# jnsquire/sregex

Hardware: AMD Instinct MI355X
Metric: GB/s input scanned (whole job), gen-data stream resident in HBM (higher is better)
Workload: dtype u8; 1 GPU; configs[1]: /[a-z]+@[a-z]+\.[a-z]+/ Pike first-match + captures; 1 stream x 4.00 GiB gen-data (abccc.. + 'aaabbccb'); bytes_per_gpu=4294967293, streams_per_gpu=1, segment_bytes=16896, fixup_rounds=0, matches=0, engine=scan, lineage_passes=0, world_size=1

## Files before the change

sregex_amd/csrc/sre_hip_batch.cpp:

```cpp
#include <sregex_hip.h>
#include "sre_hip_runtime.h"
#include "sre_hip_scan.h"
#include "sre_scan_host.h"
#include "sre_dfa.h"
#include "sre_nfa.h"
#include "sre_hip_nfa.h"
#include "sre_nfa_wide.h"
#include "sre_hip_nfa_wide.h"
#include "sre_pwave.h"
#include "sre_hip_lines.h"
#include "sre_lines_gather.h"
#include "sre_lines_route.h"
#include "sre_lines_route_key.h"
#include "sre_lines_sort.h"
#include "sre_lines_sort_text.h"
#include "sre_lines_tally.h"
#include "sre_lines_tally_top.h"
#include "sre_lines_distinct.h"
#include "sre_lines_sums.h"
#include "sre_lines_keyset.h"
#include "sre_lines_join.h"
#include "sre_hip_streams.h"
#include "sre_streams_nfa.h"
#include <stddef.h>
#include <stdio.h>
#include <stdlib.h>
#include <string.h>
#include <atomic>
#include <chrono>
#include <initializer_list>
#include <vector>

#define SRE_SPECULATIVE_FIXUPS 2

struct sre_hip_scanner_s {
    sre_program_t     *prog;
    sre_hip_program_s *dp;
    int                mode, engine;
    char               kernel_name[64];
    uint32_t           ovec_slots;
    size_t             cap_streams;
    const void       **d_ptrs;
    uint64_t          *d_lens;
    int64_t           *d_records;
    void              *d_ctx;
    size_t             ctx_stride, ctx_cap;
    uint64_t          *h_lens;
    const void       **h_ptrs;
    size_t             last_n;
    hipStream_t        last_stream;
    sre_dfa_t                *dfa;
    sre_scan_device_tables_t *tab;
    uint32_t                  seg_override;
    uint64_t                  seg_cap_env;
    sre_scan_geom_t           geom;
    uint64_t                 *d_seg_first, *h_seg_first;
    sre_seg_summary_t        *d_sum;
    sre_seg_digest_t         *d_digest;
    size_t                    sum_cap;
    sre_stream_status_t      *d_status, *h_status;
    void                     *d_acc;
    int64_t                  *d_lo, *h_lo;
    uint16_t                 *d_scratch;
    size_t                    scratch_cap;
    sre_seg_lineage_t        *d_maps, *d_blocks;
    size_t                    maps_cap;
    uint8_t                  *d_fn;
    size_t                    fn_cap;
    int                       exact_passes;
    int                       lineage_passes;
    uint32_t                  next_init_variant;
    int                       blocks_per_cu;
    hipStream_t               tail_stream;
    bool                      tail_stream_set;
    int                       fixup_rounds;
    hipEvent_t                ev0, ev1;
    int                       ev_valid;
    sre_int_t                *h_records;
    hipEvent_t                ev_done;
    uint64_t                 *d_in, *h_in;
    unsigned char            *d_out, *h_out;
    sre_nfa_t                *nfa;
    sre_nfa_tables_t          ntab;
    sre_nfa_sa_tables_t       satab;
    bool                      use_sa;
    sre_nfa_wide_t           *wnfa;
    sre_nfa_wide_tables_t     wtab;
    uint64_t                 *d_wsets;
    bool                      wide_kernel;
    struct NfaCount          *cnt;
    uint8_t                  *d_sflags, *h_sflags;
    sre_nfa_count_req_t      *d_creq, *h_creq;
    size_t                    cnt_cap;
    int                       count_rounds;
    sre_pwave_hdr_t          *h_pwave;
    void                     *d_pwave;
    size_t                    layout_n;
    sre_nfa_summary_t        *d_nsum;
    size_t                    nsum_cap;
    uint64_t                 *d_belief;
    uint8_t                  *d_bvalid;
    uint64_t                 *d_nmat;
    size_t                    nmat_cap;
    void                     *d_nacc;
    sre_nfa_status_t         *d_nstatus, *h_nstatus;
    const uint64_t           *d_eset;
    uint64_t                 *d_ends;
    size_t                    ends_cap;
    uint64_t                 *d_lblk;
    size_t                    lblk_cap;
    int64_t                  *d_rows;
    size_t                    rows_cap;
    sre_lines_info_t         *d_linfo, *h_linfo;
    bool                      last_lines;
    int                       line_batches;
    double                    lines_kernel_ms;
    bool                      lines_device;
    size_t                    short_lines;
    hipEvent_t                ev_l0, ev_l1;
    uint64_t                 *d_fval;
    size_t                    fval_cap;
    uint64_t                 *d_fblk;
    size_t                    fblk_cap;
    uint64_t                 *d_cbits;
    size_t                    cbits_cap;
    uint64_t                 *d_cblk;
    size_t                    cblk_cap;
    uint64_t                 *d_fstart;
    size_t                    fstart_cap;
    uint8_t                  *d_lit;
    uint8_t                  *h_lit;
    size_t                    lit_len;
    bool                      lit_valid;
    uint64_t                 *d_rcnt;
    size_t                    rcnt_cap;
    uint64_t                 *d_rval;
    size_t                    rval_cap;
    uint64_t                 *d_rmeta;
    size_t                    rmeta_cap;
    int32_t                  *d_rmap;
    int32_t                  *h_rmap;
    bool                      rmap_valid;
    uint64_t                 *d_rres, *h_rres;
    uint64_t                 *d_ttab;
    size_t                    ttab_cap;
    uint32_t                 *d_tslot;
    size_t                    tslot_cap;
    uint64_t                 *d_vval;
    size_t                    vval_cap;
    uint64_t                 *d_vstart;
    size_t                    vstart_cap;
    sre_ls_agg_t             *d_vcopy;
    size_t                    vcopy_cap;
    int64_t                  *d_jkey;
    size_t                    jkey_cap;
    uint64_t                 *d_kitem[2];
    size_t                    kitem_cap[2];
    int8_t                   *d_sclass;
    size_t                    sclass_cap;
    uint32_t                 *d_sline[2];
    size_t                    sline_cap[2];
    uint64_t                 *d_pcount;
    size_t                    pcount_cap;
    sre_ls_agg_t             *d_psums;
    size_t                    psums_cap;
    uint64_t                 *d_pfirst;
    size_t                    pfirst_cap;
    uint32_t                 *d_pinv;
    size_t                    pinv_cap;
    uint64_t                 *d_pstart;
    size_t                    pstart_cap;
};

struct NfaCountStream {
    const uint8_t *base;
    uint64_t       n;
    uint64_t       cur;
    uint64_t       q;
    uint64_t       horizon;
    uint32_t       var_cur, var_q, mode_q;
    int64_t        count;
    bool           done, error;
    std::vector<sre_int_t> last;
};
struct NfaCount {
    std::vector<NfaCountStream> st;
    std::vector<size_t>         active;
};

static void
scanner_release(void *data)
{
    sre_hip_scanner_t *sc = static_cast<sre_hip_scanner_t *>(data);
    delete sc->cnt;
    free(sc->h_pwave);
    if (sc->d_pwave) (void) hipFree(sc->d_pwave);
    if (sc->d_sflags) (void) hipFree(sc->d_sflags);
    if (sc->h_sflags) (void) hipHostFree(sc->h_sflags);
    if (sc->d_creq) (void) hipFree(sc->d_creq);
    if (sc->h_creq) (void) hipHostFree(sc->h_creq);
    if (sc->d_in) (void) hipFree(sc->d_in);
    if (sc->h_in) (void) hipHostFree(sc->h_in);
    if (sc->d_out) (void) hipFree(sc->d_out);
    if (sc->h_out) (void) hipHostFree(sc->h_out);
    if (sc->d_ctx) (void) hipFree(sc->d_ctx);
    if (sc->d_sum) (void) hipFree(sc->d_sum);
    if (sc->d_digest) (void) hipFree(sc->d_digest);
    if (sc->d_acc) (void) hipFree(sc->d_acc);
    if (sc->d_lo) (void) hipFree(sc->d_lo);
    if (sc->h_lo) (void) hipHostFree(sc->h_lo);
    if (sc->d_scratch) (void) hipFree(sc->d_scratch);
// ... 569 lines not shown

static uint64_t
scan_seg_knobs(sre_hip_scanner_t *sc)
{
    uint64_t seg = sc->seg_override;
    const char *e = getenv("SRE_HIP_SEG_BYTES");
    if (seg == 0 && e && atoi(e) > 0 && atoi(e) % 256 == 0) seg = (uint64_t) atoi(e);
    e = getenv("SRE_HIP_SEG_CAP");
    sc->seg_cap_env = e && atoi(e) > 0 ? (uint64_t) atoi(e) : 0;
    return seg;
}

static uint64_t
nfa_seg_knobs(sre_hip_scanner_t *sc)
{
    uint64_t seg = scan_seg_knobs(sc);
    const char *e = getenv("SRE_HIP_SEG_BYTES");
    if (seg == 0 && e && atoi(e) > 0 && atoi(e) % 64 == 0) seg = (uint64_t) atoi(e);
    return seg;
}

static uint64_t
scan_seg_cap(const sre_hip_scanner_t *sc)
{
    return sc->seg_cap_env ? sc->seg_cap_env : 40960;
}

static int
scan_events(sre_hip_scanner_t *sc)
{
    if (sc->ev0 == NULL) {
        SRE_HIP_TRY(hipEventCreate(&sc->ev0));
        SRE_HIP_TRY(hipEventCreate(&sc->ev1));
    }
    return 0;
hip_failed:
    return -1;
}

static void
call_begin(sre_hip_scanner_t *sc)
{
    sc->last_lines = false;
    sc->fixup_rounds = 0;
    sc->exact_passes = 0;
    sc->lineage_passes = 0;
    sc->ev_valid = 0;
}

static void
geom_clear(sre_hip_scanner_t *sc)
{
    sc->geom = sre_scan_geom_t();
    sc->d_eset = NULL;
}

static void
geom_device(sre_hip_scanner_t *sc, uint64_t n, uint64_t seg, uint64_t nsegs)
{
    geom_clear(sc);
    sc->geom.streams = reinterpret_cast<const uint8_t *const *>(sc->d_ptrs);
    sc->geom.lens = sc->d_lens;
    sc->geom.seg_first = sc->d_seg_first;
    sc->geom.nstreams = (uint32_t) n;
    sc->geom.seg_bytes = (uint32_t) seg;
    sc->geom.nsegs = nsegs;
}

static uint64_t
scan_resident(sre_hip_scanner_t *sc)
{
    if (sc->blocks_per_cu == 0) {
        sc->blocks_per_cu = sc->engine == SRE_HIP_ENGINE_NFA
                                ? (sc->wide_kernel ? sre_nfa_wide_blocks_per_cu(&sc->wtab)
                                   : sc->use_sa ? sre_nfa_sa_blocks_per_cu(&sc->satab)
                                              : sre_nfa_blocks_per_cu(sc->mode == SRE_HIP_THOMPSON ? 0 : 1, sc->ntab.nslices,
                                                                      sc->ntab.nassert != 0))
                                                             : sre_scan_blocks_per_cu(&sc->tab->h);
    }
    return (uint64_t) sre_hip_cu_count() * (uint64_t) sc->blocks_per_cu * SRE_SCAN_BLOCK;
}

static int scan_buffers(sre_hip_scanner_t *sc, size_t nstreams, uint64_t seg, uint64_t nsegs);

static int
nfa_buffers(sre_hip_scanner_t *sc, uint64_t nsegs)
{
    if (nsegs > sc->nsum_cap) {
        if (sc->d_nsum) (void) hipFree(sc->d_nsum);
        if (sc->d_belief) (void) hipFree(sc->d_belief);
        if (sc->d_bvalid) (void) hipFree(sc->d_bvalid);
        if (sc->d_wsets) (void) hipFree(sc->d_wsets);
        sc->d_nsum = NULL;
        sc->d_belief = NULL;
        sc->d_bvalid = NULL;
        sc->d_wsets = NULL;
        sc->nsum_cap = 0;
        SRE_HIP_TRY(hipMalloc(reinterpret_cast<void **>(&sc->d_nsum), nsegs * sizeof(sre_nfa_summary_t)));
        SRE_HIP_TRY(hipMalloc(reinterpret_cast<void **>(&sc->d_belief), nsegs * nfa_words(sc) * sizeof(uint64_t)));
        if (sc->wide_kernel) SRE_HIP_TRY(hipMalloc(reinterpret_cast<void **>(&sc->d_wsets), nsegs * 2 * nfa_words(sc) * sizeof(uint64_t)));
        SRE_HIP_TRY(hipMalloc(reinterpret_cast<void **>(&sc->d_bvalid), nsegs));
        sc->nsum_cap = nsegs;
    }
    return 0;
hip_failed:
    return -1;
}

static int
scan_geometry(sre_hip_scanner_t *sc, size_t nstreams, uint32_t init_variant, uint32_t flags, uint32_t entry_state)
{
    uint64_t total = 0;
    for (size_t i = 0; i < nstreams; i++) total += sc->h_lens[i];
    uint64_t seg = scan_seg_knobs(sc);
    if (seg == 0) {
        const uint64_t resident = scan_resident(sc);
        seg = sre_scan_auto_segment(total, resident, scan_seg_cap(sc));
    }
    uint64_t nsegs = 0;
    for (size_t i = 0; i < nstreams; i++) {
        sc->h_seg_first[i] = nsegs;
        uint64_t k = (sc->h_lens[i] + seg - 1) / seg;
        nsegs += k ? k : 1;
    }
    sc->h_seg_first[nstreams] = nsegs;
    geom_clear(sc);
    sc->geom.streams = reinterpret_cast<const uint8_t *const *>(sc->d_ptrs);
    sc->geom.lens = sc->d_lens;
    sc->geom.seg_first = sc->d_seg_first;
    sc->geom.nstreams = (uint32_t) nstreams;
    sc->geom.seg_bytes = (uint32_t) seg;
    sc->geom.nsegs = nsegs;
    sc->geom.init_variant = init_variant;
    sc->geom.entry_state = entry_state;
    sc->geom.one_ptr = static_cast<const uint8_t *>(sc->h_ptrs[0]);
    sc->geom.one_len = sc->h_lens[0];
    sc->geom.flags = flags | ((nstreams == 1 && sc->engine == SRE_HIP_ENGINE_SCAN) ? SRE_GEOM_ONE : 0u);

    if (sc->engine == SRE_HIP_ENGINE_NFA) return nfa_buffers(sc, nsegs);
    return scan_buffers(sc, nstreams, seg, nsegs);
}

static int
scan_buffers(sre_hip_scanner_t *sc, size_t nstreams, uint64_t seg, uint64_t nsegs)
{
    if (nsegs > sc->sum_cap) {
        if (sc->d_sum) (void) hipFree(sc->d_sum);
        sc->d_sum = NULL;
        sc->sum_cap = 0;
        SRE_HIP_TRY(hipMalloc(reinterpret_cast<void **>(&sc->d_sum), nsegs * sizeof(sre_seg_summary_t)));
        sc->sum_cap = nsegs;
    }
    sc->geom.digest = NULL;
    if (nsegs <= SRE_VERIFY_ONE_SEGS && sc->mode != SRE_HIP_PIKE_COUNT) {
        if (sc->d_digest == NULL
            && hipMalloc(reinterpret_cast<void **>(&sc->d_digest), SRE_VERIFY_ONE_SEGS * sizeof(sre_seg_digest_t)) != hipSuccess)
        {
            sc->d_digest = NULL;
        }
        sc->geom.digest = sc->d_digest;
    }
    {
        size_t need = nstreams * ((size_t) seg + 16);
        if (need > sc->scratch_cap) {
            if (sc->d_scratch) (void) hipFree(sc->d_scratch);
            sc->d_scratch = NULL;
            sc->scratch_cap = 0;
            SRE_HIP_TRY(hipMalloc(reinterpret_cast<void **>(&sc->d_scratch), need * sizeof(uint16_t)));
            sc->scratch_cap = need;
        }
    }
    return 0;
hip_failed:
    return -1;
}

static int
nfa_windows(sre_hip_scanner_t *sc, const int64_t *d_lo, const sre_nfa_count_req_t *d_creq, hipStream_t stream)
{
    const uint32_t n = sc->geom.nstreams;
    if (sc->d_pwave) {
        SRE_HIP_TRY(sre_launch_pike_window_wave(sc->d_pwave, sc->h_pwave, sc->d_ptrs, sc->d_lens, n, sc->d_records,
                                                sc->ovec_slots, reinterpret_cast<sre_nfa_window_t *>(sc->d_nstatus), d_lo,
                                                d_creq, stream));
    } else {
        SRE_HIP_TRY(sre_launch_pike_window(sc->dp->d_blob, sc->dp->blob_bytes, sc->d_ptrs, sc->d_lens, n, sc->d_ctx, sc->ctx_stride,
                                           sc->d_records, sc->ovec_slots,
                                           reinterpret_cast<sre_nfa_window_t *>(sc->d_nstatus), d_lo,
                                           d_creq, stream));
    }
    return 0;
hip_failed:
    return -1;
}

static int
nfa_finish(sre_hip_scanner_t *sc, const int64_t *d_lo, const sre_nfa_count_req_t *d_creq, hipStream_t stream)
{
    const int kmode = sc->mode == SRE_HIP_THOMPSON ? SRE_HIP_THOMPSON : SRE_HIP_PIKE_FIRST;
    if (sc->wide_kernel) {
        SRE_HIP_TRY(sre_launch_nfa_wide_verify(kmode, sc->wtab.W, sc->geom, sc->d_nsum, sc->d_wsets, sc->d_nacc, sc->d_nstatus,
                                               sc->d_belief, sc->d_bvalid, sc->d_records, sc->ovec_slots, d_lo, stream));
    } else {
        SRE_HIP_TRY(sre_launch_nfa_verify(kmode, sc->geom, sc->d_nsum, sc->d_nacc, sc->d_nstatus,
                                          sc->d_belief, sc->d_bvalid, sc->d_records, sc->ovec_slots, d_lo, stream));
    }
    if (sc->mode != SRE_HIP_THOMPSON) return nfa_windows(sc, d_lo, d_creq, stream);
    return 0;
hip_failed:
    return -1;
}

static uint64_t
count_horizon(uint64_t dflt)
{
    const char *e = getenv("SRE_HIP_COUNT_HORIZON");
    return e && atoll(e) > 0 ? (uint64_t) atoll(e) : dflt;
}

static int
nfa_enqueue_pass(sre_hip_scanner_t *sc, size_t nstreams, uint32_t init_variant, const uint8_t *d_sflags,
                 const sre_nfa_count_req_t *d_creq, hipStream_t stream)
{
    if (scan_geometry(sc, nstreams, init_variant, 0, 0) != 0) return -1;
    sc->geom.sflags = d_sflags;
    SRE_HIP_TRY(hipMemcpyAsync(sc->d_in, sc->h_in, (3 * sc->layout_n + 1) * sizeof(uint64_t),
                               hipMemcpyHostToDevice, stream));
    if (scan_events(sc) != 0) return -1;
    {
        const bool timed = !sc->ev_valid;
        if (timed) SRE_HIP_TRY(hipEventRecord(sc->ev0, stream));
        SRE_HIP_TRY(nfa_launch_scan(sc, NULL, NULL, NULL, stream));
        if (timed) SRE_HIP_TRY(hipEventRecord(sc->ev1, stream));
        sc->ev_valid = 1;
    }
    if (sc->tail_stream_set && sc->tail_stream != stream) {
        SRE_HIP_TRY(hipStreamWaitEvent(sc->tail_stream, sc->ev1, 0));
        stream = sc->tail_stream;
    }
    return nfa_finish(sc, NULL, d_creq, stream);
hip_failed:
    return -1;
}

static int
nfa_fixup_round(sre_hip_scanner_t *sc, const sre_nfa_count_req_t *d_creq, hipStream_t stream)
{
    if (++sc->fixup_rounds > 1000000) {
        fprintf(stderr, "[sregex-hip] NFA scanner fix-up did not converge\n");
        return -1;
    }
    if (sc->fixup_rounds > SRE_SPECULATIVE_FIXUPS && sc->geom.nsegs <= ((size_t) 1 << 23)
        && getenv("SRE_HIP_NO_NFA_EXACT") == NULL) {
        if (sc->wide_kernel) {
            const size_t need = sre_nfa_wide_matrix_bytes(sc->wtab.W, sc->geom.nsegs);
            if (need > sc->nmat_cap * 64 * sizeof(uint64_t)) {
                if (sc->d_nmat) (void) hipFree(sc->d_nmat);
                sc->d_nmat = NULL;
                sc->nmat_cap = 0;
                size_t free_b = 0, total_b = 0;
                if (hipMemGetInfo(&free_b, &total_b) == hipSuccess && need <= free_b / 2
                    && hipMalloc(reinterpret_cast<void **>(&sc->d_nmat), need) == hipSuccess) {
                    sc->nmat_cap = need / (64 * sizeof(uint64_t));
                } else {
                    (void) hipGetLastError();
                    sc->d_nmat = NULL;
                }
            }
            if (sc->d_nmat) {
                SRE_HIP_TRY(sre_launch_nfa_wide_exact_entries(sc->wtab, sc->geom, sc->d_nsum, sc->d_wsets, sc->d_lo, sc->d_nmat,
                                                              sc->d_belief, sc->d_bvalid, stream));
                sc->exact_passes++;
            }
        } else {
            if (sc->geom.nsegs > sc->nmat_cap) {
                if (sc->d_nmat) (void) hipFree(sc->d_nmat);
                sc->d_nmat = NULL;
                sc->nmat_cap = 0;
                SRE_HIP_TRY(hipMalloc(reinterpret_cast<void **>(&sc->d_nmat), sc->geom.nsegs * 64 * sizeof(uint64_t)));
                sc->nmat_cap = sc->geom.nsegs;
            }
            SRE_HIP_TRY(sre_launch_nfa_exact_entries(sc->use_sa ? 1 : 0, sc->ntab, sc->satab, sc->geom, sc->d_nsum, sc->d_lo,
                                                     sc->d_nmat, sc->d_belief, sc->d_bvalid, stream));
            sc->exact_passes++;
        }
    }
    SRE_HIP_TRY(nfa_launch_scan(sc, sc->d_lo, sc->d_belief, sc->d_bvalid, stream));
    return nfa_finish(sc, sc->d_lo, d_creq, stream);
hip_failed:
    return -1;
}

static int
nfa_settle(sre_hip_scanner_t *sc, size_t n, const sre_nfa_count_req_t *d_creq, hipStream_t stream, bool *psettled)
{
    for (bool first = true;; first = false) {
        if (!first) {
            SRE_HIP_TRY(hipMemcpyAsync(sc->h_nstatus, sc->d_nstatus, n * sizeof(sre_nfa_status_t),
                                       hipMemcpyDeviceToHost, stream));
            SRE_HIP_TRY(hipStreamSynchronize(stream));
        }
        size_t pending = 0;
        for (size_t i = 0; i < n; i++) {
            if (sc->h_nstatus[i].done) {
                sc->h_lo[i] = -1;
            } else {
                sc->h_lo[i] = sc->h_nstatus[i].first_bad;
                pending++;
            }
        }
        if (pending == 0) break;
// ... 240 lines not shown
    return -1;
}

typedef uint64_t sre_lines_info_t::*LinfoWord;
#define LINFO(word) (&sre_lines_info_t::word)

static hipError_t
linfo_read(sre_hip_scanner_t *sc, hipStream_t stream, std::initializer_list<LinfoWord> words)
{
    const char *base = reinterpret_cast<const char *>(sc->h_linfo);
    size_t      lo = sizeof(sre_lines_info_t), hi = 0;
    for (LinfoWord w : words) {
        const size_t at = (size_t) (reinterpret_cast<const char *>(&(sc->h_linfo->*w)) - base);
        lo = at < lo ? at : lo;
        hi = at + sizeof(uint64_t) > hi ? at + sizeof(uint64_t) : hi;
    }
    return hipMemcpyAsync(reinterpret_cast<char *>(sc->h_linfo) + lo, reinterpret_cast<const char *>(sc->d_linfo) + lo, hi - lo,
                          hipMemcpyDeviceToHost, stream);
}

static int
lines_status_counters(sre_hip_scanner_t *sc, size_t n, hipStream_t stream)
{
    SRE_HIP_TRY(sre_launch_lines_settle(sc->d_status, (uint32_t) n, sc->d_linfo, stream));
    SRE_HIP_TRY(linfo_read(sc, stream, {LINFO(pending), LINFO(maps)}));
    SRE_HIP_TRY(hipStreamSynchronize(stream));
    return 0;
hip_failed:
    return -1;
}

static int
scan_settle(sre_hip_scanner_t *sc, size_t n, hipStream_t stream, bool with_captures, bool *psettled,
            bool counters = false)
{
    bool settled = true;
    int  batch = sc->mode == SRE_HIP_PIKE_COUNT ? 2 : SRE_SPECULATIVE_FIXUPS + 1;
    for (;;) {
        size_t pending = 0;
        if (counters) pending = (size_t) sc->h_linfo->pending;
        else for (size_t i = 0; i < n; i++) pending += sc->h_status[i].done ? 0 : 1;
        if (pending == 0) break;
        settled = false;
        for (int r = 0; r < batch; r++) {
            if (++sc->fixup_rounds > 1000000) {
                fprintf(stderr, "[sregex-hip] scanner fix-up did not converge\n");
                return -1;
            }
            const uint8_t *d_entry = NULL;
            static const bool count_exact = getenv("SRE_HIP_NO_COUNT_EXACT") == NULL;
            if ((sc->mode != SRE_HIP_PIKE_COUNT || count_exact) && sc->fixup_rounds > SRE_SPECULATIVE_FIXUPS) {
                if (sc->geom.nsegs > sc->fn_cap) {
                    if (sc->d_fn) (void) hipFree(sc->d_fn);
                    sc->d_fn = NULL;
                    sc->fn_cap = 0;
                    const size_t nchunks = sc->geom.nsegs / 256 + 1;
                    SRE_HIP_TRY(hipMalloc(reinterpret_cast<void **>(&sc->d_fn),
                                          sc->geom.nsegs * 64 + nchunks * 64 + nchunks + sc->geom.nsegs + 64));
                    sc->fn_cap = sc->geom.nsegs;
                }
                const size_t nchunks = sc->geom.nsegs / 256 + 1;
                uint8_t *d_comp = sc->d_fn + sc->geom.nsegs * 64, *d_chunk = d_comp + nchunks * 64;
                uint8_t *d_ent = d_chunk + nchunks;
                SRE_HIP_TRY(sre_launch_exact_entries(sc->tab->d_tab, sc->tab->h, sc->geom, sc->d_sum, sc->d_status,
                                                     sc->d_fn, d_comp, d_chunk, d_ent, stream));
                d_entry = d_ent;
                sc->exact_passes++;
            }
            SRE_HIP_TRY(sre_launch_scan(sc->tab->d_tab, sc->tab->h, sc->geom, sc->d_sum, sc->d_status, d_entry, stream));
            SRE_HIP_TRY(sre_launch_verify(sc->tab->h, sc->geom, sc->d_sum, sc->d_acc, sc->d_status, stream));
            if (with_captures) {
                SRE_HIP_TRY(sre_launch_captures(sc->tab->d_tab, sc->tab->h, sc->geom, sc->d_sum,
                                                sc->d_status, sc->d_scratch, sc->d_records,
                                                sc->ovec_slots, NULL, NULL, 0, 0, stream));
            }
        }
        if (counters) {
            if (lines_status_counters(sc, n, stream) != 0) return -1;
        } else {
            SRE_HIP_TRY(hipMemcpyAsync(sc->h_status, sc->d_status, n * sizeof(sre_stream_status_t),
                                       hipMemcpyDeviceToHost, stream));
            SRE_HIP_TRY(hipStreamSynchronize(stream));
        }
        batch = sc->mode == SRE_HIP_PIKE_COUNT ? (batch < 16 ? 2 * batch : 16) : 1;
    }
    if (psettled) *psettled = settled;
    return 0;
hip_failed:
    return -1;
}

static int
scan_lineage_pass(sre_hip_scanner_t *sc, hipStream_t stream)
{
    if (sc->geom.nsegs > sc->maps_cap) {
        if (sc->d_maps) (void) hipFree(sc->d_maps);
        if (sc->d_blocks) (void) hipFree(sc->d_blocks);
        sc->d_maps = sc->d_blocks = NULL;
        sc->maps_cap = 0;
        SRE_HIP_TRY(hipMalloc(reinterpret_cast<void **>(&sc->d_maps),
                              sc->geom.nsegs * sizeof(sre_seg_lineage_t)));
        SRE_HIP_TRY(hipMalloc(reinterpret_cast<void **>(&sc->d_blocks),
                              (sc->geom.nsegs / SRE_LINEAGE_BLOCK + 1) * sizeof(sre_seg_lineage_t)));
        sc->maps_cap = sc->geom.nsegs;
    }
    sc->lineage_passes++;
    SRE_HIP_TRY(sre_launch_lineage(sc->tab->d_tab, sc->tab->h, sc->geom, sc->d_sum,
                                   sc->d_status, sc->d_maps, sc->d_blocks, stream));
    SRE_HIP_TRY(sre_launch_captures(sc->tab->d_tab, sc->tab->h, sc->geom, sc->d_sum,
                                    sc->d_status, sc->d_scratch, sc->d_records,
                                    sc->ovec_slots, sc->d_maps, sc->d_blocks,
                                    1, 0, stream));
    return 0;
hip_failed:
    return -1;
}

extern "C" SRE_API int
sre_hip_scan_results(sre_hip_scanner_t *sc, sre_int_t *results)
{
    if (sc->last_lines) return -1;
    if (sc->last_n == 0) return 0;
    const size_t n = sc->last_n;
    hipStream_t  stream = sc->last_stream;

    const size_t bytes = n * (2 + (size_t) sc->ovec_slots) * sizeof(int64_t);
    bool         settled = true;

    if (sc->engine == SRE_HIP_ENGINE_NFA && sc->cnt != NULL) return nfa_count_rounds(sc, results);
    SRE_HIP_TRY(hipEventSynchronize(sc->ev_done));
    if (sc->engine == SRE_HIP_ENGINE_NFA && nfa_settle(sc, n, NULL, stream, &settled) != 0) return -1;
    if (sc->engine == SRE_HIP_ENGINE_SCAN) {
        if (scan_settle(sc, n, stream, true, &settled) != 0) return -1;
        if (sc->mode != SRE_HIP_THOMPSON) {
            size_t want = 0;
            for (size_t i = 0; i < n; i++) want += sc->h_status[i].need_maps != 0;
            if (want) {
                settled = false;
                if (scan_lineage_pass(sc, stream) != 0) return -1;
            }
        }
    }
    if (sc->engine == SRE_HIP_ENGINE_SCAN && getenv("SRE_HIP_DEBUG_STATUS")) {
        for (size_t i = 0; i < n && i < 8; i++) {
            const sre_stream_status_t &t = sc->h_status[i];
            fprintf(stderr, "[sregex-hip] stream %zu: rc %lld count %lld ev_pos %lld ev_sp %lld ev_state %u ev_sym %u "
                            "ev_apos %lld ev_astate %u ev_seg %lld limit %lld need_maps %d seg %u\n",
                    i, (long long) t.rc, (long long) t.count, (long long) t.ev_pos, (long long) t.ev_sp,
                    t.ev_state, t.ev_sym, (long long) t.ev_apos, t.ev_astate, (long long) t.ev_seg,
                    (long long) t.limit, t.need_maps, sc->geom.seg_bytes);
        }
        const size_t ns = sc->geom.nsegs < 16 ? (size_t) sc->geom.nsegs : 16;
        std::vector<sre_seg_summary_t> hs(ns);
        if (hipMemcpy(hs.data(), sc->d_sum, ns * sizeof(sre_seg_summary_t), hipMemcpyDeviceToHost) == hipSuccess) {
            for (size_t k = 0; k < ns; k++) {
                fprintf(stderr, "[sregex-hip]   seg %zu: s_in %x s_out %x flags %x count %lld cur_sp %lld term %lld "
                                "pe_pos %lld lm_pos %lld lm_sp %lld\n",
                        k, hs[k].s_in, hs[k].s_out, hs[k].flags, (long long) hs[k].count,
                        (long long) hs[k].cur_sp, (long long) hs[k].term_pos, (long long) hs[k].pe_pos,
                        (long long) hs[k].lm_pos, (long long) hs[k].lm_sp);
            }
        }
    }
    if (!settled) {
        SRE_HIP_TRY(hipMemcpyAsync(sc->h_records, sc->d_records, bytes, hipMemcpyDeviceToHost, stream));
        if (sc->engine == SRE_HIP_ENGINE_NFA) {
            SRE_HIP_TRY(hipMemcpyAsync(sc->h_nstatus, sc->d_nstatus, n * sizeof(sre_nfa_status_t),
                                       hipMemcpyDeviceToHost, stream));
        }
        SRE_HIP_TRY(hipStreamSynchronize(stream));
    }
    memcpy(results, sc->h_records, bytes);
    return 0;
hip_failed:
    return -1;
}

extern "C" SRE_API int
sre_hip_scan_batch(sre_hip_scanner_t *sc, const void *const *d_streams, const size_t *lens,
    size_t nstreams, sre_int_t *results, void *hip_stream)
{
    if (sre_hip_scan_enqueue(sc, d_streams, lens, nstreams, hip_stream) != 0) return -1;
    return sre_hip_scan_results(sc, results);
}


template <typename T>
static int
lines_grow(T **p, size_t *cap, size_t bytes)
{
    if (bytes <= *cap) return 0;
    if (*p) (void) hipFree(*p);
    *p = NULL;
    *cap = 0;
    SRE_HIP_TRY(hipMalloc(reinterpret_cast<void **>(p), bytes));
    *cap = bytes;
    return 0;
hip_failed:
    return -1;
}

static uint64_t
lines_batch_limit(void)
{
    const char     *e = getenv("SRE_HIP_LINES_BATCH");
    const long long v = e ? atoll(e) : 0;
    return v > 0 ? (v < (1ll << 24) ? (uint64_t) v : (uint64_t) 1 << 24) : SRE_LINES_BATCH;
}

static int
lines_split(sre_hip_scanner_t *sc, const void *d_buf, size_t len, int delim, hipStream_t stream, uint64_t *pn)
{
    *pn = 0;
    if (len == 0) return 0;
    const uint64_t head = reinterpret_cast<uintptr_t>(d_buf) & 15u;
    const uint64_t ntiles = (head + len + SRE_LINES_TILE_BYTES - 1) / SRE_LINES_TILE_BYTES;
    const uint64_t nblk = (lines_batch_limit() + SRE_LINES_ITEMS - 1) / SRE_LINES_ITEMS + 1;
    if (lines_grow(&sc->d_lblk, &sc->lblk_cap, (ntiles > nblk ? ntiles : nblk) * sizeof(uint64_t)) != 0) return -1;
    SRE_HIP_TRY(sre_launch_lines_count(d_buf, len, (uint32_t) delim, sc->d_lblk, sc->d_linfo, stream));
    SRE_HIP_TRY(hipMemcpyAsync(&sc->h_linfo->nlines, &sc->d_linfo->nlines, sizeof(uint64_t), hipMemcpyDeviceToHost, stream));
    SRE_HIP_TRY(hipStreamSynchronize(stream));
    if (lines_grow(&sc->d_ends, &sc->ends_cap, sc->h_linfo->nlines * sizeof(uint64_t)) != 0) return -1;
    SRE_HIP_TRY(sre_launch_lines_write(d_buf, len, (uint32_t) delim, sc->d_lblk, sc->d_ends, stream));
    *pn = sc->h_linfo->nlines;
    return 0;
hip_failed:
    return -1;
}

struct LinesSink {
    int        delim;
    void      *d_out;
    size_t     out_cap;
    sre_int_t *d_index;
    size_t     index_cap;
    int        mode;
    const sre_extract_groups_t *groups;
    int                         fsep;
    const sre_subst_pieces_t   *pieces;
    bool                        route;
    uint32_t                    nreg;
    const sre_extract_groups_t *vgroups;
    bool                        context;
    const uint64_t             *d_cbits;
    uint32_t                    join;
    const void                 *d_dict;
};

static bool
sink_open(LinesSink *sink, const sre_hip_scanner_t *sc, const void *d_buf, size_t len, int delim, int flags, void *d_out,
          size_t out_cap, sre_int_t *d_index, size_t index_cap)
{
    if (sc == NULL || delim < 0 || delim > 255 || (out_cap != 0 && d_out == NULL) || (index_cap != 0 && d_index == NULL)
        || (len != 0 && d_buf == NULL))
    {
        return false;
    }
    if (len != 0 && out_cap != 0) {
        const uintptr_t b = reinterpret_cast<uintptr_t>(d_buf), o = reinterpret_cast<uintptr_t>(d_out);
        if (o < b + len && b < o + out_cap) return false;
    }
    *sink = LinesSink();
    sink->delim = sink->fsep = delim;
    sink->mode = (flags & SRE_HIP_LINES_ALL) ? 2 : (flags & SRE_HIP_LINES_INVERT) ? 1 : 0;
    sink->d_out = d_out;
    sink->out_cap = out_cap;
    sink->d_index = d_index;
    sink->index_cap = index_cap;
    return true;
}

static bool
sink_first_match(const sre_hip_scanner_t *sc, const char *call, const char *reads)
{
    if (sc->mode == SRE_HIP_PIKE_FIRST) return true;
    fprintf(stderr, "[sregex-hip] %s: the scanner's mode must be SRE_HIP_PIKE_FIRST (the first match's %s)\n", call, reads);
    return false;
}

static bool
sink_groups(const sre_hip_scanner_t *sc, const int *groups, size_t ngroups, sre_extract_groups_t *gr)
{
    memset(gr, 0, sizeof(*gr));
    gr->k = (uint32_t) ngroups;
    for (size_t f = 0; f < ngroups; f++) {
        if (groups[f] < 0 || groups[f] > 0xFFFF || 2 * (size_t) groups[f] + 1 >= (size_t) sc->ovec_slots) return false;
        gr->g[f] = (uint16_t) groups[f];
    }
    return true;
}

static uint32_t
sink_entries(const LinesSink *sink)
{
    return sink->pieces ? sink->pieces->np + 2 : sink->groups ? sink->groups->k : sink->join ? sink->join : 1;
}

static int
sink_select(sre_hip_scanner_t *sc, const LinesSink *sink, uint32_t slots, uint64_t nmax, uint64_t i0, hipStream_t stream)
{
    const int64_t          *recs = sc->d_records;
    const uint64_t         *ends = sc->d_ends;
    const sre_lines_info_t *li = sc->d_linfo;
    uint64_t               *val = sc->d_fval, *start = sc->d_fstart;
    const int               all = sink->mode == 2;
    if (sink->route) SRE_HIP_TRY(sre_launch_route_select(recs, slots, nmax, i0, sink->nreg, sc->d_rmap, ends, li, val, stream));
    else if (sink->pieces) SRE_HIP_TRY(sre_launch_subst_select(recs, slots, nmax, i0, all, sink->pieces, ends, li, val, start, stream));
// ... 2187 lines not shown
```

sregex_amd/csrc/sre_hip_scan.h:

```cpp
#ifndef SRE_HIP_SCAN_H
#define SRE_HIP_SCAN_H

#include <hip/hip_runtime.h>
#include <stdint.h>

#define SRE_CEILING_GRID   2048

#include "sre_scan_fast.h"

#define SRE_SCAN_MAX_SHADOWS  2u
#define SRE_SCAN_MAX_ROWS(bits)   ((65536u - 768u - ((bits) == 8 ? 512u : (8u / (bits)) * 512u)) / 1024u)
#define SRE_SCAN_MAX_STATES       62u
#define SRE_SCAN_BLOCK        256u
#define SRE_SCAN_LDS_LIMIT    (128u * 1024u)
#define SRE_CAPTURE_MAX_GRID   16384u
#define SRE_CAPTURE_LANE_STREAMS 4096u
#define SRE_CAPTURE_LDS_LIMIT  (144u * 1024u)
#define SRE_SCAN_ROUND        64u
#define SRE_SCAN_LINE         128u
#define SRE_SCAN_SEG_ALIGN    256u

#define SRE_SCAN_NINIT 4u
#define SRE_DEV_EV_DONE_EMPTY 3
#define SRE_DEV_EV_POP_FULL   4

typedef struct {
    uint32_t next;
    uint8_t  kind;
    uint8_t  src;
    uint16_t regex;
    uint32_t lin_off;
    uint16_t lin_n;
    uint8_t  skipped;
    uint8_t  pad;
    uint64_t saves;
    uint64_t early;
} sre_dev_trans_t;

typedef struct {
    uint32_t nstates, ncls, nslots, max_threads;
    uint32_t init[4];
    uint32_t word_restart;
    int32_t  mode;
    uint32_t fast_bytes;
    uint32_t stride, class_bits;
    const uint32_t        *fast;
    const uint32_t        *fast_plain;
    const uint8_t         *cls;
    const sre_dev_trans_t *trans;
    const uint16_t        *trans2;
    const uint8_t         *lin_parent;
    const uint64_t        *lin_saves;
    const uint64_t        *lin_early;
    const uint8_t         *lin_flags;
    uint32_t               lin_total, list_total;
    const uint8_t         *state_flags;
    const uint32_t        *list_off;
    const uint32_t        *list_pcs;
    const uint32_t        *multi_ncaps;
    uint32_t nregexes;
    uint32_t any_fresh;
    uint32_t nshadow;
    uint32_t fast_rows;
    uint32_t wide;
    uint8_t  shadow_state[SRE_SCAN_MAX_SHADOWS];
    const uint8_t         *unskip;
    const uint16_t        *neutral;
} sre_scan_tables_t;

typedef struct {
    uint32_t s_in;
    uint32_t s_out;
    uint32_t flags;
    uint32_t pad;
    uint32_t pe_state, pe_sym;
    int64_t  pe_pos, pe_sp;
    uint32_t lm_state, lm_sym;
    int64_t  lm_pos, lm_sp;
    int64_t  lm_apos, pe_apos;
    uint32_t lm_astate, pe_astate;
    int64_t  term_pos;
    int64_t  count;
    int64_t  cur_sp;
    int64_t  in_pe_pos;
    uint32_t in_pe_state, in_pe_sym;
    uint32_t stable_until, stable_from;
} sre_seg_summary_t;

typedef struct sre_seg_digest_s {
    uint32_t s_in, s_out, bits, count;
} sre_seg_digest_t;

#define SRE_SUM_PENDING   1u
#define SRE_SUM_TERM      2u
#define SRE_SUM_LASTEV    4u
#define SRE_SUM_ERROR     8u
#define SRE_SUM_IN_PENDING 16u
#define SRE_SUM_STABLE    32u

#define SRE_STATE_SKIP    0x40000000u

typedef struct {
    uint64_t anc;
    uint16_t saved;
    uint16_t stop;
    uint32_t pad;
} sre_seg_lineage_t;

#define SRE_LINEAGE_BLOCK  256u
#define SRE_WALK_BUDGET    256

#define SRE_STREAM_MAX_THREADS 64u
#define SRE_STREAM_MAX_SLOTS   64u
typedef struct {
    uint32_t state;
    uint32_t has_pending;
    int64_t  pending_regex;
    int64_t  pending_vec[SRE_STREAM_MAX_SLOTS];
    int64_t  caps[SRE_STREAM_MAX_THREADS][SRE_STREAM_MAX_SLOTS];
    int64_t  caps_next[SRE_STREAM_MAX_THREADS][SRE_STREAM_MAX_SLOTS];
} sre_stream_ctx_t;

#define SRE_VERIFY_ONE_SEGS 8192u
#define SRE_STREAM_UNSETTLED (-100)
#define SRE_STREAM_PENDING   (-101)

typedef struct {
    int64_t  rc;
    int64_t  has_pending, pending[2];
    int64_t  ev_in_chunk;
    int64_t  poisoned;
    int64_t  next_state;
    int64_t  ev_slot1;
    int64_t  ov[SRE_STREAM_MAX_SLOTS];
} sre_stream_result_t;

typedef struct {
    int64_t  first_bad;
    int64_t  limit;
    int64_t  count;
    int64_t  rc;
    int64_t  ev_pos, ev_sp;
    uint32_t ev_state, ev_sym;
    int64_t  ev_apos;
    uint32_t ev_astate;
    uint32_t valid_from;
    int64_t  ev_seg;
    int64_t  unst_seg;
    int64_t  unst_end;
    int32_t  done;
    int32_t  error;
    int32_t  need_maps;
    int32_t  pad;
} sre_stream_status_t;

typedef struct {
    const uint8_t *const *streams;
    const uint64_t *lens;
    const uint64_t *seg_first;
    uint32_t nstreams;
    uint32_t seg_bytes;
    uint64_t nsegs;
    uint32_t init_variant;
    uint32_t flags;
    uint32_t entry_state;
    const uint8_t *one_ptr;
    uint64_t one_len;
    const uint8_t *sflags;
    struct sre_seg_digest_s *digest;
    const uint32_t *sentry;
} sre_scan_geom_t;
#define SRE_SENTRY_STATE(e)   ((e) & 0xffffu)
#define SRE_SENTRY_CONTINUES  0x40000000u
#define SRE_SENTRY_NO_EOF     0x80000000u
#define SRE_SFLAG_INIT(f)    ((f) & 3u)
#define SRE_SFLAG_SNAP(f)    (((f) >> 2) & 3u)
#define SRE_SFLAG_MODE(f)    (((f) >> 4) & 1u)
#define SRE_SFLAG_NO_EOF     32u

#define SRE_GEOM_CONTINUES 1u
#define SRE_GEOM_NO_EOF    2u
#define SRE_GEOM_ONE       4u

#ifdef __HIPCC__
static __host__ __device__ inline uint64_t
sre_scan_auto_segment(uint64_t total, uint64_t resident, uint64_t seg_cap)
{
    uint64_t rounds = (total + resident * seg_cap - 1) / (resident * seg_cap);
    if (rounds < 1) rounds = 1;
    const uint64_t lanes = resident * rounds - (resident * rounds >> 6);
    uint64_t       seg = (total / lanes + SRE_SCAN_SEG_ALIGN) / SRE_SCAN_SEG_ALIGN * SRE_SCAN_SEG_ALIGN;
    if (seg < 256) seg = 256;
    if (seg % 4096 == 0) seg += SRE_SCAN_SEG_ALIGN;
    return seg;
}

static __device__ inline const uint8_t *
geom_ptr(const sre_scan_geom_t &G, uint32_t s)
{
    return (G.flags & SRE_GEOM_ONE) ? G.one_ptr : G.streams[s];
}
static __device__ inline uint64_t
geom_len(const sre_scan_geom_t &G, uint32_t s)
{
    return (G.flags & SRE_GEOM_ONE) ? G.one_len : G.lens[s];
}
static __device__ inline uint64_t
geom_first(const sre_scan_geom_t &G, uint32_t i)
{
    return (G.flags & SRE_GEOM_ONE) ? (i ? G.nsegs : 0) : G.seg_first[i];
}
#endif

#ifdef __cplusplus
extern "C" {
#endif
hipError_t sre_launch_gen_data(void *d_dst, uint64_t n, uint64_t tail_len, const void *d_tail,
    hipStream_t stream);
hipError_t sre_launch_read_ceiling(const void *d_src, uint64_t n, uint32_t *d_sink,
    hipStream_t stream);
hipError_t sre_launch_read_pattern(const void *d_src, uint64_t n, uint32_t seg_bytes,
    uint32_t tile, uint32_t lds_bytes, uint32_t *d_sink, hipStream_t stream);

size_t sre_scan_lds_bytes(const sre_scan_tables_t *h_tab);
int sre_scan_blocks_per_cu(const sre_scan_tables_t *h_tab);

hipError_t sre_launch_scan(const sre_scan_tables_t *d_tab, sre_scan_tables_t h_tab,
    sre_scan_geom_t geom, sre_seg_summary_t *d_sum, const sre_stream_status_t *d_lo, const uint8_t *d_entry,
    hipStream_t stream);
hipError_t sre_launch_exact_entries(const sre_scan_tables_t *d_tab, sre_scan_tables_t h_tab,
    sre_scan_geom_t geom, const sre_seg_summary_t *d_sum, const sre_stream_status_t *d_status,
    uint8_t *d_fn, uint8_t *d_comp, uint8_t *d_chunk_entry, uint8_t *d_entry, hipStream_t stream);
hipError_t sre_launch_stream_tail(const sre_scan_tables_t *d_tab, sre_scan_tables_t h_tab,
    sre_scan_geom_t geom, const sre_seg_summary_t *d_sum, sre_stream_status_t *d_status,
    uint16_t *d_scratch, sre_stream_ctx_t *d_ctx, sre_stream_result_t *result, int64_t base, int eof,
    uint32_t ovec_slots, int verify, hipStream_t stream);
hipError_t sre_launch_upload_words(const uint64_t *h_src_mapped, uint64_t *d_dst, uint32_t nwords, hipStream_t stream);
size_t sre_scan_verify_acc_bytes(uint32_t nstreams);
hipError_t sre_scan_verify_acc_init(void *d_acc, uint32_t nstreams, hipStream_t stream);
hipError_t sre_launch_verify(sre_scan_tables_t h_tab, sre_scan_geom_t geom,
    const sre_seg_summary_t *d_sum, void *d_acc, sre_stream_status_t *d_status,
    hipStream_t stream);
hipError_t sre_launch_captures(const sre_scan_tables_t *d_tab, sre_scan_tables_t h_tab,
    sre_scan_geom_t geom, const sre_seg_summary_t *d_sum, sre_stream_status_t *d_status,
    uint16_t *d_scratch, int64_t *d_records, uint32_t ovec_slots,
    const sre_seg_lineage_t *d_maps, const sre_seg_lineage_t *d_blocks, int use_maps,
    int verify, hipStream_t stream);
hipError_t sre_launch_lineage(const sre_scan_tables_t *d_tab, sre_scan_tables_t h_tab,
    sre_scan_geom_t geom, const sre_seg_summary_t *d_sum, const sre_stream_status_t *d_status,
    sre_seg_lineage_t *d_maps, sre_seg_lineage_t *d_blocks, hipStream_t stream);
#ifdef __cplusplus
// ... 4 lines not shown
```

sregex_amd/csrc/sre_hip_scan.hip:

```cpp
#include <hip/hip_runtime.h>
#include <stdlib.h>
#include "sre_hip_scan.h"
#include "sre_hip_streams.h"
#include "sre_hip_tile.h"

#define SRE_HIP_PIKE_COUNT 2
#define EV_DONE 1
#define EV_POP  2
#define RC_DECLINED (-5)
#define RC_ERROR    (-1)


__global__ void
sre_k_gen_data(uint8_t *__restrict__ dst, uint64_t n, uint64_t body, const uint8_t *__restrict__ tail)
{
    const uint64_t stride = (uint64_t) gridDim.x * blockDim.x * 16;
    for (uint64_t base = ((uint64_t) blockIdx.x * blockDim.x + threadIdx.x) * 16; base < n;
         base += stride)
    {
        uint8_t  v[16];
        unsigned ph = (unsigned) (base % 5);
#pragma unroll
        for (int k = 0; k < 16; k++) {
            uint64_t i = base + k;
// ... 302 lines not shown
            const bool    empty = w.ev_kind == EV_POP || w.ev_kind == SRE_DEV_EV_DONE_EMPTY;
            const int64_t e = pop ? w.ev_pos : w.ev_pos + 1;
            w.complete_match();
            if (empty) {
                if (e >= w.n) {
                    w.term_pos = p;
                    w.fl |= F_FINISHED;
                    return;
                }
                w.cur_sp = e + 1;
            } else {
                w.cur_sp = e;
            }
            w.st = T.init[restart_variant_of(T, byte_at(w.cur_sp - 1))];
            p = w.cur_sp;
            if (p > p_to && p_to <= w.n) w.fl |= F_SKIP_NEXT;
            w.anchor_pos = -1;
        }
    }
}

struct SpanResult {
    int64_t  sp;
    int64_t  last_pos, last_sp;
    uint32_t last_state, last_sym;
    int64_t  pend_pos;
    uint32_t pend_state, pend_sym;
};

__device__ __attribute__((noinline)) SpanResult
resolve_fast_span(const sre_scan_tables_t *Tp, const uint16_t *tr2, const uint8_t *data, int64_t gpos,
                  uint32_t len, uint32_t s0, int64_t sp0, int64_t pend0_pos, uint32_t pend0_state, uint32_t pend0_sym)
{
    const sre_scan_tables_t &T = *Tp;
    SpanResult r;
    uint32_t   st = s0;
    r.sp = sp0;
    r.last_pos = r.last_sp = -1;
    r.last_state = r.last_sym = 0;
    r.pend_pos = pend0_pos;
    r.pend_state = pend0_state;
    r.pend_sym = pend0_sym;
    for (uint32_t b = 0; b < len; b++) {
        const uint32_t         sym = T.cls[data[gpos + b]];
        const uint32_t t2 = tr2[st * (T.ncls + 1) + sym];
        struct { uint32_t next; uint8_t kind; } tr = {t2 & 0xffu, (uint8_t) (t2 >> 8)};
        if (tr.kind && tr.next == 0) {
            const bool pop = tr.kind == SRE_DEV_EV_POP_FULL && gpos + b > 0;
            r.last_pos = gpos + b;
            r.last_state = st;
            r.last_sym = sym;
            r.last_sp = r.sp;
            r.sp = pop ? gpos + b : gpos + b + 1;
            r.pend_pos = -1;
            st = T.init[restart_variant(T, data, r.sp)];
            if (pop) st = tr2[st * (T.ncls + 1) + sym] & 0xffu;
        } else if (tr.kind) {
            r.pend_pos = gpos + b;
            r.pend_state = st;
            r.pend_sym = sym;
            st = tr.next;
        } else if (tr.next == 0 && gpos + b > 0) {
            r.last_pos = r.pend_pos;
            r.last_state = r.pend_state;
            r.last_sym = r.pend_sym;
            r.last_sp = r.sp;
            r.sp = gpos + b;
            st = T.init[restart_variant(T, data, r.sp)];
            const uint32_t t3 = tr2[st * (T.ncls + 1) + sym];
            r.pend_pos = -1;
            if ((t3 >> 8) && (t3 & 0xffu) == 0) {
                r.last_pos = gpos + b;
                r.last_state = st;
                r.last_sym = sym;
                r.last_sp = r.sp;
                r.sp = gpos + b + 1;
                st = T.init[restart_variant(T, data, r.sp)];
            } else {
                if (t3 >> 8) {
                    r.pend_pos = gpos + b;
                    r.pend_state = st;
                    r.pend_sym = sym;
                }
                st = t3 & 0xffu;
            }
        } else {
            st = tr.next;
        }
    }
    return r;
}

template <int H>
__device__ inline uint32_t
add_w0_w(uint32_t a, uint32_t b)
{
    uint32_t r;
    if (H == 0) asm("v_add_u32_sdwa %0, %1, %2 dst_sel:DWORD dst_unused:UNUSED_PAD src0_sel:WORD_0 src1_sel:WORD_0" : "=v"(r) : "v"(a), "v"(b));
    if (H == 1) asm("v_add_u32_sdwa %0, %1, %2 dst_sel:DWORD dst_unused:UNUSED_PAD src0_sel:WORD_0 src1_sel:WORD_1" : "=v"(r) : "v"(a), "v"(b));
    if (H == 2) asm("v_add_u32_sdwa %0, %1, %2 dst_sel:DWORD dst_unused:UNUSED_PAD src0_sel:WORD_0 src1_sel:DWORD" : "=v"(r) : "v"(a), "v"(b));
    return r;
}

__device__ inline uint32_t
add_b3(uint32_t a, uint32_t b)
{
    uint32_t r;
    asm("v_add_u32_sdwa %0, %1, %2 dst_sel:DWORD dst_unused:UNUSED_PAD src0_sel:DWORD src1_sel:BYTE_3" : "=v"(r) : "v"(a), "v"(b));
    return r;
}

template <int K>
__device__ inline uint32_t
byte_x4(uint32_t v, uint32_t sh)
{
    uint32_t r;
    if (K == 0) asm("v_lshlrev_b32_sdwa %0, %1, %2 dst_sel:DWORD dst_unused:UNUSED_PAD src0_sel:DWORD src1_sel:BYTE_0" : "=v"(r) : "v"(sh), "v"(v));
    if (K == 1) asm("v_lshlrev_b32_sdwa %0, %1, %2 dst_sel:DWORD dst_unused:UNUSED_PAD src0_sel:DWORD src1_sel:BYTE_1" : "=v"(r) : "v"(sh), "v"(v));
    if (K == 2) asm("v_lshlrev_b32_sdwa %0, %1, %2 dst_sel:DWORD dst_unused:UNUSED_PAD src0_sel:DWORD src1_sel:BYTE_2" : "=v"(r) : "v"(sh), "v"(v));
    if (K == 3) asm("v_lshlrev_b32_sdwa %0, %1, %2 dst_sel:DWORD dst_unused:UNUSED_PAD src0_sel:DWORD src1_sel:BYTE_3" : "=v"(r) : "v"(sh), "v"(v));
    return r;
}

#ifdef SRE_NO_TAIL_PRIO
#define SRE_TAIL_PRIO() ((void) 0)
#else
#define SRE_TAIL_PRIO() __builtin_amdgcn_s_setprio(3)
#endif

#ifndef SRE_SCAN_PREFETCH
#define SRE_SCAN_PREFETCH 1
#endif
#ifndef SRE_SCAN_SPLIT_HOLD
#define SRE_SCAN_SPLIT_HOLD 3
#endif
constexpr int
scan_split_of(int mode, int bits, bool wide, bool grow)
{
#ifdef SRE_SCAN_SPLIT
    (void) mode; (void) bits; (void) wide; (void) grow;
    return SRE_SCAN_SPLIT;
#else
    if (mode != SRE_HIP_PIKE_COUNT) return (bits == 2 || bits == 4) ? 4 : 1;
    return (bits == 4 && !wide && grow) ? 4 : 1;
#endif
}
#ifndef SRE_FIRST_BLOCKS
#define SRE_FIRST_BLOCKS 4
#endif
#ifndef SRE_COUNT_BLOCKS
#define SRE_COUNT_BLOCKS 3
#endif

template <int MODE, int BITS, bool WIDE, bool GROW>
__global__ __launch_bounds__(SRE_SCAN_BLOCK, MODE == SRE_HIP_PIKE_COUNT ? SRE_COUNT_BLOCKS : SRE_FIRST_BLOCKS) void
sre_k_scan(const sre_scan_tables_t *__restrict__ tabp, sre_scan_geom_t G,
           sre_seg_summary_t *__restrict__ sum, const sre_stream_status_t *__restrict__ st_lo,
           const uint8_t *__restrict__ entry)
{
    constexpr int      TILE = SRE_SCAN_ROUND;
    constexpr int      WARM = SRE_SCAN_LINE;
    constexpr int      STRIDE = 8 / BITS;
    constexpr uint32_t ROWRAW = TILE / STRIDE * (WIDE ? 2 : 1);
    constexpr uint32_t ROWB = 2 * ROWRAW + 16;
    constexpr int      GIDX = 16 / STRIDE;
    typedef const __attribute__((address_space(3))) uint32_t *lds_u32_t;
    extern __shared__ __attribute__((aligned(16))) uint8_t lds[];
    __shared__ uint16_t clsx[BITS == 8 ? 1 : 8 / BITS][256];
    __shared__ sre_scan_tables_t Ts;

    const uint32_t tid = threadIdx.x;
    const uint32_t nst = tabp->nstates, nrows = tabp->fast_rows, nsh = tabp->nshadow;
    uint32_t *fast = reinterpret_cast<uint32_t *>(lds);
    uint8_t  *clsl = lds + nrows * SRE_FAST_ROW_BYTES;
    uint8_t  *trl = clsl + 256;
    const uint32_t tr_bytes = (nst * (tabp->ncls + 1) * 2u + 15u) & ~15u;
    uint8_t  *sfl = trl + tr_bytes;
    uint8_t  *tile = lds + (((size_t) (sfl - lds) + nst + 15u) & ~(size_t) 15u);
    RowDesc  *rows = reinterpret_cast<RowDesc *>(tile + SRE_SCAN_BLOCK * ROWB);
    (void) nrows;
    if (tid == 0) {
        Ts = *tabp;
        Ts.cls = clsl;
        Ts.state_flags = sfl;
    }
    constexpr uint32_t LDS_SLOW = 1u << 16;
    constexpr uint32_t LDS_CNT_SHIFT = 24;
    constexpr uint32_t LDS_FRESH = 1u << 17;
    const uint32_t fast_lds = (uint32_t) (uintptr_t) (__attribute__((address_space(3))) uint8_t *) lds;
    const uint32_t trap_lds = fast_lds + nst * SRE_FAST_ROW_BYTES;
    const uint32_t shadow_lds = trap_lds + SRE_FAST_ROW_BYTES;
    auto to_lds = [fast_lds, trap_lds](uint32_t g) -> uint32_t {
        if (g & SRE_FAST_SLOW) return trap_lds | LDS_SLOW;
        return (fast_lds + (g & ~(SRE_FAST_ROW_BYTES - 1)))
               | (((g >> SRE_FAST_CNT_SHIFT) & SRE_FAST_CNT_MASK) << LDS_CNT_SHIFT)
               | ((MODE == SRE_HIP_PIKE_COUNT && (g & SRE_FAST_EVT)) ? (128u << LDS_CNT_SHIFT) : 0u)
               | ((MODE == SRE_HIP_PIKE_COUNT && (g & SRE_FAST_NEXT_FRESH)) ? LDS_FRESH : 0u);
    };
    for (uint32_t i = tid; i < nst * 64; i += SRE_SCAN_BLOCK) {
        uint4 e = reinterpret_cast<const uint4 *>(tabp->fast)[i];
        e.x = to_lds(e.x);
        e.y = to_lds(e.y);
        e.z = to_lds(e.z);
        e.w = to_lds(e.w);
        reinterpret_cast<uint4 *>(fast)[i] = e;
    }
    fast[nst * 256 + tid] = trap_lds | LDS_SLOW;
    for (uint32_t q = 0; q < nsh; q++) {
        const uint32_t s = tabp->shadow_state[q], addr = shadow_lds + q * SRE_FAST_ROW_BYTES;
        const uint32_t gl = tabp->fast[s * 256 + tid];
        fast[(nst + 1 + q) * 256 + tid] = (gl & SRE_FAST_STABLE) ? addr : to_lds(gl);
    }
    for (uint32_t i = tid; i < nst * (tabp->ncls + 1); i += SRE_SCAN_BLOCK) {
        reinterpret_cast<uint16_t *>(trl)[i] = tabp->trans2[i];
    }
    for (uint32_t i = tid; i < tabp->nstates; i += SRE_SCAN_BLOCK) sfl[i] = tabp->state_flags[i];
    clsl[tid] = tabp->cls[tid];
    if (BITS != 8) {
#pragma unroll
        for (int u = 0; u < 8 / BITS; u++) clsx[u][tid] = (uint16_t) ((uint32_t) tabp->cls[tid] << (BITS * u + (WIDE ? 2 : 0)));
    }
    __syncthreads();
    const sre_scan_tables_t &T = Ts;

    const uint64_t g = (uint64_t) blockIdx.x * SRE_SCAN_BLOCK + tid;
    bool           active = g < G.nsegs;
    uint32_t       sidx = 0;
    uint64_t       k = 0;
    int64_t        lo_s = -2;
    if (active) {
        uint32_t a = 0, b = G.nstreams;
        while (b - a > 1) {
            uint32_t m = (a + b) >> 1;
            if (geom_first(G, m) <= g) a = m; else b = m;
        }
        sidx = a;
        k = g - geom_first(G, a);
        if (st_lo != nullptr) {
            lo_s = st_lo[sidx].done ? -1 : st_lo[sidx].first_bad;
            if (lo_s < 0 || (int64_t) k < lo_s) active = false;
        }
    }

    Walk w;
    w.T = &T;
    w.tr2 = reinterpret_cast<const uint16_t *>(trl);
    w.data = nullptr;
    w.n = 0;
    w.st = 0;
    w.ev_kind = 0;
    w.ev_state = w.ev_sym = 0;
    w.ev_pos = w.ev_sp = -1;
    w.ev_apos = -1;
    w.ev_astate = 0;
    w.cur_sp = -1;
    w.warm_lo = 0;
    w.anchor_pos = -1;
    w.anchor_state = 0;
    w.lm_state = w.lm_sym = 0;
    w.lm_pos = w.lm_sp = w.lm_apos = -1;
    w.lm_astate = 0;
    w.count = 0;
    w.term_pos = -1;
    w.fl = 0;

    int64_t  seg_a = 0, seg_b = 0;
    uint32_t s_in = 0, seed = 0;
    int64_t  in_pe_pos = -1;
    uint32_t in_pe_state = 0, in_pe_sym = 0;
    bool     last_seg = false, warm = false;
    RowDesc mine;
    mine.addr = 0;
    mine.lo = 0;
    mine.hi16 = -1;
    if (active) {
        w.data = geom_ptr(G, sidx);
        w.n = (int64_t) geom_len(G, sidx);
        seg_a = (int64_t) k * G.seg_bytes;
        seg_b = seg_a + G.seg_bytes;
        const uint64_t nseg = geom_first(G, sidx + 1) - geom_first(G, sidx);
        last_seg = (k + 1 == nseg);
        if (seg_b > w.n) seg_b = w.n;
        if (last_seg && G.sentry != nullptr && (G.sentry[sidx] & SRE_SENTRY_NO_EOF)) w.fl |= F_NO_EOF;

        if (k == 0) {
            w.st = G.sentry != nullptr ? SRE_SENTRY_STATE(G.sentry[sidx])
                   : (G.flags & SRE_GEOM_CONTINUES) ? G.entry_state : T.init[G.init_variant];
            w.cur_sp = 0;
        } else if (lo_s >= 0 && (int64_t) k == lo_s) {
            const sre_seg_summary_t &c = sum[g - 1];
            w.st = c.s_out & ~SRE_STATE_SKIP;
            w.set(F_SKIP_NEXT, MODE == SRE_HIP_PIKE_COUNT && (c.s_out & SRE_STATE_SKIP) != 0);
            w.cur_sp = c.cur_sp;
            if (c.flags & SRE_SUM_PENDING) {
                w.fl |= F_HAS_EV;
                w.ev_state = c.pe_state;
                w.ev_sym = c.pe_sym;
                w.ev_pos = c.pe_pos;
                w.ev_sp = c.pe_sp;
                w.ev_apos = c.pe_apos;
                w.ev_astate = c.pe_astate;
                w.ev_kind = (uint8_t) (w.tr2[c.pe_state * (T.ncls + 1) + c.pe_sym] >> 8);
                if (MODE == SRE_HIP_PIKE_COUNT) {
                    w.fl |= F_IN_PENDING;
                    in_pe_pos = c.pe_pos;
                    in_pe_state = c.pe_state;
                    in_pe_sym = c.pe_sym;
                }
            }
        } else if (entry != nullptr && entry[g] != 0xffu) {
            w.st = entry[g];
            if (MODE == SRE_HIP_PIKE_COUNT && lo_s > 0 && (T.state_flags[w.st] & 1)) {
                const sre_seg_summary_t &c = sum[geom_first(G, sidx) + lo_s - 1];
                if (c.flags & SRE_SUM_PENDING) {
                    w.fl |= F_HAS_EV | F_IN_PENDING;
                    w.ev_state = c.pe_state;
                    w.ev_sym = c.pe_sym;
                    w.ev_pos = c.pe_pos;
                    w.ev_sp = c.pe_sp;
                    w.ev_apos = -1;
                    w.ev_astate = 0;
                    w.ev_kind = (uint8_t) (w.tr2[c.pe_state * (T.ncls + 1) + c.pe_sym] >> 8);
                    in_pe_pos = c.pe_pos;
                    in_pe_state = c.pe_state;
                    in_pe_sym = c.pe_sym;
                }
            }
        } else {
            warm = true;
            seed = T.init[0];
            if (lo_s > 0) {
                const sre_seg_summary_t &c = sum[geom_first(G, sidx) + lo_s - 1];
                const uint32_t           cs = c.s_out & ~SRE_STATE_SKIP;
                if (cs != 0) {
                    if (!(MODE == SRE_HIP_PIKE_COUNT && (T.state_flags[cs] & 1))) {
                        seed = cs;
                    } else if (c.flags & SRE_SUM_PENDING) {
                        seed = cs;
                        w.fl |= F_HAS_EV;
                        w.ev_state = c.pe_state;
                        w.ev_sym = c.pe_sym;
                        w.ev_pos = c.pe_pos;
                        w.ev_sp = c.pe_sp;
                        w.ev_apos = -1;
                        w.ev_astate = 0;
                        w.ev_kind = (uint8_t) (w.tr2[c.pe_state * (T.ncls + 1) + c.pe_sym] >> 8);
                    }
                }
            }
            w.st = seed;
        }
        w.warm_lo = seg_a >= (int64_t) WARM ? seg_a - (int64_t) WARM : 0;
        s_in = w.st | (MODE == SRE_HIP_PIKE_COUNT && w.f(F_SKIP_NEXT) ? SRE_STATE_SKIP : 0u);
        mine.addr = (uint64_t) reinterpret_cast<uintptr_t>(w.data) + (uint64_t) (seg_a - WARM);
        mine.lo = warm ? (seg_a >= WARM ? 0 : (int32_t) (WARM - seg_a)) : WARM;
        mine.hi16 = (int32_t) (WARM + (seg_b - seg_a)) - 16;
    }
    rows[tid] = mine;

    int64_t  fcA_pos = -1, fcB_pos = -1, fc_sp0 = -1;
    uint32_t fcA_len = 0, fcA_s0 = 0, fcB_len = 0, fcB_s0 = 0;
    int64_t  lz_pos = -1;
    uint32_t lz_s0 = 0;
    auto note_span = [&](int64_t pos, uint32_t len, uint32_t s0, uint32_t cnt, bool warm_round) {
        w.fl &= ~F_HAS_EV;
        if (warm_round) return;
        if (w.f(F_SP_DIRTY)) {
            fcA_pos = fcB_pos;
            fcA_len = fcB_len;
            fcA_s0 = fcB_s0;
        } else {
            fc_sp0 = w.cur_sp;
            fcA_pos = -1;
        }
        fcB_pos = pos;
        fcB_len = len;
        fcB_s0 = s0;
        if (w.f(F_PEND_LAZY)) {
            fcB_pos = lz_pos;
            fcB_len = len + (w.f(F_LZ_GROUP) ? 16u : (uint32_t) TILE);
            fcB_s0 = lz_s0;
        }
        w.fl |= F_SP_DIRTY;
        w.count += cnt;
    };
    constexpr bool any_fresh = GROW;
    auto fast_span_done = [&](int64_t pos, uint32_t len, uint32_t s0, uint32_t sum, bool fresh1, bool warm_round) {
        if (!any_fresh) {
            if (sum) note_span(pos, len, s0, sum, warm_round);
            return;
        }
        if (sum == 0) {
            w.fl &= ~F_PEND_LAZY;
            return;
        }
        if (sum & 127u) note_span(pos, len, s0, sum & 127u, warm_round);
        else if (sum) w.fl &= ~F_HAS_EV;
        if (fresh1) {
            w.fl |= F_PEND_LAZY;
            w.set(F_LZ_GROUP, len == 16u);
            lz_pos = pos;
            lz_s0 = s0;
        } else {
            w.fl &= ~F_PEND_LAZY;
        }
    };
    auto settle = [&]() {
        if (MODE != SRE_HIP_PIKE_COUNT || !(w.fl & (F_SP_DIRTY | F_PEND_LAZY))) return;
        if (w.f(F_SP_DIRTY)) {
            int64_t sp0 = fc_sp0;
            if (fcA_pos >= 0) sp0 = resolve_fast_span(&T, w.tr2, w.data, fcA_pos, fcA_len, fcA_s0, -1, -1, 0, 0).sp;
            const SpanResult r = resolve_fast_span(&T, w.tr2, w.data, fcB_pos, fcB_len, fcB_s0, sp0, w.ev_pos, w.ev_state, w.ev_sym);
            if (r.last_pos >= 0) {
                w.fl |= F_LM_VALID;
                w.lm_pos = r.last_pos;
                w.lm_state = r.last_state;
                w.lm_sym = r.last_sym;
                w.lm_sp = r.last_sp;
                const bool anchored = r.last_sp < fcB_pos && r.last_pos - fcB_pos <= 256 && fcB_pos >= seg_a;
                w.lm_apos = anchored ? fcB_pos : (int64_t) -1;
                w.lm_astate = anchored ? fcB_s0 : 0u;
            }
            w.cur_sp = r.sp;
            w.fl &= ~F_SP_DIRTY;
        }
        if (w.f(F_PEND_LAZY)) {
            const SpanResult r = resolve_fast_span(&T, w.tr2, w.data, lz_pos, w.f(F_LZ_GROUP) ? 16u : (uint32_t) TILE, lz_s0,
                                                   -1, -1, 0, 0);
            w.fl &= ~F_PEND_LAZY;
            if (r.pend_pos >= 0) {
                w.fl |= F_HAS_EV;
                w.ev_pos = r.pend_pos;
                w.ev_state = r.pend_state;
                w.ev_sym = r.pend_sym;
                w.ev_kind = (uint8_t) (w.tr2[r.pend_state * (T.ncls + 1) + r.pend_sym] >> 8);
                w.ev_sp = w.cur_sp;
                const bool anchored = w.cur_sp < lz_pos && lz_pos >= seg_a;
                w.ev_apos = anchored ? lz_pos : (int64_t) -1;
                w.ev_astate = anchored ? lz_s0 : 0u;
            }
        }
    };

    constexpr uint32_t SU_UNSET = 0xffffffffu;
    uint32_t           su = SU_UNSET, run_off = 0;
    static_assert(SRE_SCAN_MAX_SHADOWS == 2, "two shadow rows");
    const uint32_t sh_st0 = nsh > 0 ? tabp->shadow_state[0] : 0xffffu, sh_st1 = nsh > 1 ? tabp->shadow_state[1] : 0xffffu;
    const uint32_t sh_ad0 = shadow_lds, sh_ad1 = shadow_lds + SRE_FAST_ROW_BYTES;
    const uint32_t     two = 2;
    (void) two;

    const uint32_t nrounds = WARM / TILE + G.seg_bytes / TILE;
    const uint32_t lag = (tid >> 5) & 1u;
    constexpr uint32_t DIST = SRE_SCAN_PREFETCH;
    constexpr int      NLOOK = TILE * BITS / 8;
    constexpr int      SPLIT = scan_split_of(MODE, BITS, WIDE, GROW);
    static_assert(SPLIT == 1 || SPLIT == 2 || SPLIT == 4, "SRE_SCAN_SPLIT is 1, 2 or 4");
    uint32_t           hold = 0;
    __syncthreads();
    auto round = [&](const uint32_t s, uint4 (&regs)[4]) __attribute__((always_inline)) {
        if (SPLIT > 1) {
            if (__builtin_amdgcn_ballot_w64((w.fl & F_SPLIT_MISS) != 0)) {
                hold = SRE_SCAN_SPLIT_HOLD;
                w.fl &= ~F_SPLIT_MISS;
            } else if (hold) {
                hold--;
            }
        }
        __builtin_amdgcn_fence(__ATOMIC_ACQ_REL, "wavefront");
        __builtin_amdgcn_wave_barrier();
        tile_store<BITS, WIDE>(regs, tile, clsx, tid, s);
        __builtin_amdgcn_fence(__ATOMIC_ACQ_REL, "wavefront");
        __builtin_amdgcn_wave_barrier();
        if (s + DIST <= nrounds) tile_fetch(regs, rows, tid, s + DIST);

        if (s < lag || s - lag >= nrounds) return;
        const uint32_t r = s - lag;
        const bool     warm_round = (r < WARM / TILE);
        if (!active || w.f(F_FINISHED) || (warm_round && !warm)) return;
        const int64_t base = seg_a - WARM + (int64_t) r * TILE;
        if (base >= seg_b || base < 0) return;
        w.anchor_pos = warm_round ? -1 : base;
        w.anchor_state = w.st;

        constexpr int ROWW = (ROWRAW + 3) / 4;
// ... 79 lines not shown
                        uint32_t nv = 1;
                        t = tc[0];
                        cnt = cc[0];
#pragma unroll
                        for (int c = 1; c < SPLIT; c++) {
                            if (nv == (uint32_t) c && ((t ^ t0) & 0xffffu) == 0) {
                                t = tc[c];
                                cnt += cc[c];
                                nv = c + 1;
                            }
                        }
                        if (!(t & LDS_SLOW)) {
#pragma unroll
                            for (int c = 1; c < SPLIT; c++) {
                                if (nv <= (uint32_t) c) serial(c * L, (c + 1) * L);
                            }
                        }
                    }
                }
            } else {
                serial(0, NLOOK);
            }
            if (!(t & LDS_SLOW)) {
                const uint32_t ridx = ((t & 0xffffu) - fast_lds) / SRE_FAST_ROW_BYTES;
                if (MODE == SRE_HIP_PIKE_COUNT) fast_span_done(base, TILE, w.st, cnt, (t & LDS_FRESH) != 0, warm_round);
                w.st = MODE == SRE_HIP_PIKE_COUNT ? ridx : ridx <= nst ? ridx : ridx == nst + 1 ? sh_st0 : sh_st1;
                if (MODE != SRE_HIP_PIKE_COUNT && w.f(F_SHADOW) && ridx <= nst) {
                    w.fl &= ~F_SHADOW;
                    if (su == SU_UNSET) su = (uint32_t) (base - seg_a);
                }
                if (r + 1 == WARM / TILE) {
                    s_in = w.st | (MODE == SRE_HIP_PIKE_COUNT && w.f(F_SKIP_NEXT) ? SRE_STATE_SKIP : 0u);
                    settle();
                    w.cur_sp = -1;
                    if (w.f(F_HAS_EV)) w.ev_sp = -1;
                    if (w.st == 0) w.fl |= F_FINISHED;
                    if (MODE == SRE_HIP_PIKE_COUNT) {
                        w.set(F_IN_PENDING, w.f(F_HAS_EV));
                        in_pe_pos = w.ev_pos;
                        in_pe_state = w.ev_state;
                        in_pe_sym = w.ev_sym;
                    }
                }
                return;
            }
        }
        if (MODE != SRE_HIP_PIKE_COUNT && !warm_round) {
            w.fl &= ~F_SHADOW;
            if (su == SU_UNSET) su = (uint32_t) (base - seg_a);
        }
#pragma unroll 1
        for (uint32_t q = 0; q < TILE / 16; q++) {
            const int64_t gp = base + q * 16;
            if (gp >= seg_b || w.f(F_FINISHED)) break;
            const int64_t g_end = gp + 16 <= seg_b ? gp + 16 : seg_b;
            bool          exact = (g_end != gp + 16) || (MODE == SRE_HIP_PIKE_COUNT && w.f(F_SKIP_NEXT));
            uint32_t      t = fast_lds + w.st * SRE_FAST_ROW_BYTES, cnt = 0;
            if (!exact) {
                constexpr int GW = GIDX * (WIDE ? 2 : 1) / 4;
                uint32_t      gw[GW];
                const uint32_t *gsrc = reinterpret_cast<const uint32_t *>(tile + tid * ROWB + (r & 1u) * ROWRAW) + q * GW;
#pragma unroll
                for (int x = 0; x < GW; x++) gw[x] = gsrc[x];
#pragma unroll
                for (int j = 0; j < GIDX; j++) {
                    const uint32_t ix = WIDE ? (gw[j >> 1] >> ((j & 1) * 16)) & 0xffffu
                                             : ((gw[j >> 2] >> ((j & 3) * 8)) & 0xffu) << 2;
                    t = *(lds_u32_t) (uintptr_t) ((t & 0xffffu) + ix);
                    if (MODE == SRE_HIP_PIKE_COUNT) cnt += t >> LDS_CNT_SHIFT;
                }
                exact = (t & LDS_SLOW) != 0;
            }
            if (exact) {
                settle();
                slow_run<MODE>(w, gp, g_end, warm_round, seed);
            } else {
                const uint32_t st1 = ((t & 0xffffu) - fast_lds) / SRE_FAST_ROW_BYTES;
                if (MODE == SRE_HIP_PIKE_COUNT) fast_span_done(gp, 16, w.st, cnt, (t & LDS_FRESH) != 0, warm_round);
                w.st = st1;
            }
        }
        if (r + 1 == WARM / TILE) {
            s_in = w.st | (MODE == SRE_HIP_PIKE_COUNT && w.f(F_SKIP_NEXT) ? SRE_STATE_SKIP : 0u);
            settle();
            w.cur_sp = -1;
            if (w.f(F_HAS_EV)) w.ev_sp = -1;
            if (w.st == 0) w.fl |= F_FINISHED;
            if (MODE == SRE_HIP_PIKE_COUNT) {
                w.set(F_IN_PENDING, w.f(F_HAS_EV));
                in_pe_pos = w.ev_pos;
                in_pe_state = w.ev_state;
                in_pe_sym = w.ev_sym;
            }
        }
    
    };
    uint4 regs[4];
    tile_fetch(regs, rows, tid, 0);
    if (DIST == 1) {
        for (uint32_t s = 0; s <= nrounds; s++) round(s, regs);
    } else {
        uint4 regs2[4];
        if (nrounds >= 1) tile_fetch(regs2, rows, tid, 1);
        for (uint32_t s = 0; s <= nrounds; s += 2) {
            round(s, regs);
            if (s + 1 <= nrounds) round(s + 1, regs2);
        }
    }

    if (!active) return;

    if (last_seg && !w.f(F_FINISHED) && !(G.flags & SRE_GEOM_NO_EOF) && !w.f(F_NO_EOF)) {
        settle();
        w.anchor_pos = -1;
        slow_run<MODE>(w, w.n, w.n + 1, false, 0);
    }
    settle();

    sre_seg_summary_t out;
    {
        const uint32_t seg_len = (uint32_t) (seg_b - seg_a);
        if (MODE == SRE_HIP_PIKE_COUNT || (w.f(F_FINISHED) && su == SU_UNSET)) su = 0;
        out.stable_until = su == SU_UNSET ? seg_len : su;
        out.stable_from = (MODE != SRE_HIP_PIKE_COUNT && w.f(F_SHADOW)) ? run_off : seg_len;
    }
    out.s_in = w.f(F_UNRESOLVED) ? 0xffffffffu : s_in;
    out.s_out = w.st | (MODE == SRE_HIP_PIKE_COUNT && w.f(F_SKIP_NEXT) ? SRE_STATE_SKIP : 0u);
    out.flags = 0;
    out.pad = 0;
    out.count = w.count;
    out.term_pos = w.term_pos;
    out.cur_sp = w.cur_sp;
    if (w.f(F_FINISHED) && w.term_pos >= 0) out.flags |= SRE_SUM_TERM;
    if (w.f(F_ERROR)) out.flags |= SRE_SUM_ERROR;
    if (w.f(F_HAS_EV)) out.flags |= SRE_SUM_PENDING;
    if (w.f(F_LM_VALID)) out.flags |= SRE_SUM_LASTEV;
    if (MODE == SRE_HIP_PIKE_COUNT && w.f(F_IN_PENDING)) out.flags |= SRE_SUM_IN_PENDING;
    if (MODE != SRE_HIP_PIKE_COUNT && out.stable_until == G.seg_bytes && !last_seg) out.flags |= SRE_SUM_STABLE;
    out.in_pe_pos = in_pe_pos;
    out.in_pe_state = in_pe_state;
    out.in_pe_sym = in_pe_sym;
    out.pe_state = w.ev_state;
    out.pe_sym = w.ev_sym;
    out.pe_pos = w.ev_pos;
    out.pe_sp = w.ev_sp;
    out.lm_state = w.lm_state;
    out.lm_sym = w.lm_sym;
    out.lm_pos = w.lm_pos;
    out.lm_sp = w.lm_sp;
    out.lm_apos = w.lm_apos;
    out.lm_astate = w.lm_astate;
    out.pe_apos = w.ev_apos;
    out.pe_astate = w.ev_astate;
    sum[g] = out;
    if (MODE != SRE_HIP_PIKE_COUNT && G.digest != nullptr) {
        sre_seg_digest_t dg;
        dg.s_in = out.s_in;
        dg.s_out = out.s_out;
        dg.bits = ((out.flags & SRE_SUM_TERM) ? 2u : 0u) | ((out.flags & SRE_SUM_LASTEV) ? 4u : 0u) | (out.cur_sp >= 0 ? 8u : 0u)
                  | ((out.flags & SRE_SUM_STABLE) ? 0u : 16u);
        dg.count = (uint32_t) out.count;
        G.digest[g] = dg;
    }
}


#define SRE_FN_CHUNK 256u

template <int BITS>
__global__ __launch_bounds__(256) void
sre_k_seg_functions(const sre_scan_tables_t *__restrict__ tabp, sre_scan_geom_t G,
                    const sre_stream_status_t *__restrict__ status, uint8_t *__restrict__ fn)
{
    constexpr int STRIDE = 8 / BITS;
    constexpr int GIDX = 16 / STRIDE;
    typedef const __attribute__((address_space(3))) uint32_t *lds_u32_t;
    extern __shared__ __attribute__((aligned(16))) uint8_t lds[];
    __shared__ uint16_t clsx[BITS == 8 ? 1 : 8 / BITS][256];
    const uint32_t tid = threadIdx.x, nst = tabp->nstates, nsym = tabp->ncls + 1;
    uint32_t *fast = reinterpret_cast<uint32_t *>(lds);
    uint8_t  *clsl = lds + (nst + 1) * SRE_FAST_ROW_BYTES;
    uint16_t *tr2 = reinterpret_cast<uint16_t *>(clsl + 256);
    constexpr uint32_t LDS_SLOW = 1u << 16;
    const uint32_t fast_lds = (uint32_t) (uintptr_t) (__attribute__((address_space(3))) uint8_t *) lds;
    const uint32_t trap_lds = fast_lds + nst * SRE_FAST_ROW_BYTES;
    for (uint32_t i = tid; i < nst * 256; i += 256) {
        const uint32_t gl = tabp->fast[i];
        fast[i] = (gl & SRE_FAST_SLOW) ? (trap_lds | LDS_SLOW) : fast_lds + (gl & ~(SRE_FAST_ROW_BYTES - 1));
    }
    fast[nst * 256 + tid] = trap_lds | LDS_SLOW;
    clsl[tid] = tabp->cls[tid];
    for (uint32_t i = tid; i < nst * nsym; i += 256) tr2[i] = tabp->trans2[i];
    if (BITS != 8) {
#pragma unroll
        for (int u = 0; u < 8 / BITS; u++) clsx[u][tid] = (uint16_t) ((uint32_t) tabp->cls[tid] << (BITS * u + 2));
    }
    __syncthreads();

    const uint32_t lane = tid & 63u;
    const uint64_t g = (uint64_t) blockIdx.x * 4 + (tid >> 6);
    if (g >= G.nsegs) return;
    const uint32_t s = stream_of(G, g);
    const uint64_t k = g - geom_first(G, s);
    if (status[s].done || (int64_t) k < status[s].first_bad) return;
    if (lane >= nst) {
        fn[g * 64 + lane] = 0;
        return;
    }
    const uint8_t *data = geom_ptr(G, s);
    const int64_t  n = (int64_t) geom_len(G, s);
    int64_t        p = (int64_t) k * G.seg_bytes, seg_b = p + G.seg_bytes;
    if (seg_b > n) seg_b = n;
    uint32_t cur = lane;
    const bool count_mode = tabp->mode == SRE_HIP_PIKE_COUNT;
    auto exact = [&](int64_t from, int64_t to) {
        if (!count_mode) {
            for (int64_t q = from; q < to; q++) cur = tr2[cur * nsym + clsl[data[q]]] & 0xffu;
            return;
        }
        int64_t  pend = -1;
        uint32_t pkind = 0, guard = 0;
        for (int64_t q = from; q < to; q++) {
            const uint32_t sym = clsl[data[q]];
            const uint32_t t2 = tr2[cur * nsym + sym];
            if (t2 >> 8) {
                pend = q;
                pkind = t2 >> 8;
            }
            cur = t2 & 0xffu;
            if (cur != 0) continue;
            int64_t sp = q + 1;
            if (pend >= 0) {
                const bool    pop = pkind == EV_POP || pkind == SRE_DEV_EV_POP_FULL;
                const bool    empty = pkind == EV_POP || pkind == SRE_DEV_EV_DONE_EMPTY;
                const int64_t e = pop ? pend : pend + 1;
                sp = empty ? e + 1 : e;
            } else if (++guard < 2) {
                sp = q;
            }
            if (pend >= 0) guard = 0;
            if (sp < 1) sp = 1;
            if (sp > n) sp = n;
            cur = tabp->init[restart_variant_of(*tabp, data[sp - 1])];
            pend = -1;
            q = sp - 1;
        }
    };
    for (; p + 16 <= seg_b; p += 16) {
        const sre_u32x4 v = *reinterpret_cast<const __attribute__((address_space(1))) sre_u32x4_unaligned *>(
            reinterpret_cast<uintptr_t>(data + p));
        const uint32_t words[4] = {v.x, v.y, v.z, v.w};
        uint32_t       t = fast_lds + cur * SRE_FAST_ROW_BYTES;
#pragma unroll
        for (int j = 0; j < GIDX; j++) {
            uint32_t ix = 0;
#pragma unroll
            for (int u = 0; u < STRIDE; u++) {
                const int      b = j * STRIDE + u;
                const uint32_t c = (words[b >> 2] >> ((b & 3) * 8)) & 0xffu;
                ix |= BITS == 8 ? c << 2 : (uint32_t) clsx[u][c];
            }
            t = *(lds_u32_t) (uintptr_t) ((t & 0xffffu) + ix);
        }
        if (t & LDS_SLOW) exact(p, p + 16);
        else cur = ((t & 0xffffu) - fast_lds) / SRE_FAST_ROW_BYTES;
    }
    exact(p, seg_b);
    fn[g * 64 + lane] = (uint8_t) cur;
}

__global__ __launch_bounds__(64) void
sre_k_fn_chunks(uint64_t nsegs, const uint8_t *__restrict__ fn, uint8_t *__restrict__ comp)
{
    const uint64_t c = blockIdx.x;
    uint32_t       v = threadIdx.x;
    const uint64_t g0 = c * SRE_FN_CHUNK, g1 = g0 + SRE_FN_CHUNK <= nsegs ? g0 + SRE_FN_CHUNK : nsegs;
    for (uint64_t g = g0; g < g1; g++) v = fn[g * 64 + (v & 63u)];
    comp[c * 64 + threadIdx.x] = (uint8_t) v;
}

__global__ void
sre_k_fn_resolve(sre_scan_geom_t G, const sre_seg_summary_t *__restrict__ sum,
                 const sre_stream_status_t *__restrict__ status, const uint8_t *__restrict__ fn,
                 const uint8_t *__restrict__ comp, uint8_t *__restrict__ entry, uint8_t *__restrict__ chunk_entry)
{
    const uint32_t s = blockIdx.x * blockDim.x + threadIdx.x;
    if (s >= G.nstreams || status[s].done || status[s].first_bad < 1) return;
    const uint64_t first = geom_first(G, s), g_hi = geom_first(G, s + 1);
    uint64_t       g = first + (uint64_t) status[s].first_bad;
    uint32_t       v = sum[g - 1].s_out & 63u;
    while (g < g_hi) {
        if (g % SRE_FN_CHUNK == 0 && g + SRE_FN_CHUNK <= g_hi) {
            chunk_entry[g / SRE_FN_CHUNK] = (uint8_t) v;
            v = comp[(g / SRE_FN_CHUNK) * 64 + v];
            g += SRE_FN_CHUNK;
        } else {
            entry[g] = (uint8_t) v;
            v = fn[g * 64 + v];
            g++;
        }
    }
}

__global__ void
sre_k_fn_fill(uint64_t nsegs, const uint8_t *__restrict__ fn, const uint8_t *__restrict__ chunk_entry,
              uint8_t *__restrict__ entry)
{
    const uint64_t c = (uint64_t) blockIdx.x * blockDim.x + threadIdx.x;
    if (c * SRE_FN_CHUNK >= nsegs || chunk_entry[c] == 0xffu) return;
    uint32_t v = chunk_entry[c];
    for (uint64_t g = c * SRE_FN_CHUNK; g < (c + 1) * SRE_FN_CHUNK && g < nsegs; g++) {
        entry[g] = (uint8_t) v;
        v = fn[g * 64 + (v & 63u)];
    }
}


struct VerifyAcc {
    unsigned long long bad, end;
    unsigned long long count, evseg, spseg;
    unsigned long long unst;
    unsigned long long unst_end;
};

__global__ __launch_bounds__(256) void
sre_k_verify_a(sre_scan_geom_t G, const sre_seg_summary_t *__restrict__ sum, VerifyAcc *__restrict__ acc,
               int mode)
{
    SRE_TAIL_PRIO();
    const uint64_t g = (uint64_t) blockIdx.x * blockDim.x + threadIdx.x;
    const bool     valid = g < G.nsegs;
    const uint32_t s = stream_of(G, valid ? g : G.nsegs - 1);
    unsigned long long kb = ~0ull, ke = ~0ull;
    if (valid) {
        const uint64_t k = g - geom_first(G, s);
        const uint32_t s_in = sum[g].s_in;
        bool           bad = s_in == 0xffffffffu;
        if (k > 0) {
            const sre_seg_summary_t &p = sum[g - 1], &c = sum[g];
            if (s_in != p.s_out) bad = true;
            if (mode == SRE_HIP_PIKE_COUNT) {
                const bool pp = (p.flags & SRE_SUM_PENDING) != 0, cp = (c.flags & SRE_SUM_IN_PENDING) != 0;
                if (pp != cp) bad = true;
                if (pp && cp && (p.pe_pos != c.in_pe_pos || p.pe_state != c.in_pe_state || p.pe_sym != c.in_pe_sym)) {
                    bad = true;
                }
            }
        }
        if (bad) kb = k;
        if (sum[g].flags & SRE_SUM_TERM) ke = k;
    }
    const uint32_t s0 = (uint32_t) __builtin_amdgcn_readfirstlane((int) s);
    if (__builtin_amdgcn_ballot_w64(s != s0) == 0) {
        for (int d = 32; d >= 1; d >>= 1) {
            const unsigned long long ob = __shfl_xor(kb, d, 64), oe = __shfl_xor(ke, d, 64);
            kb = ob < kb ? ob : kb;
            ke = oe < ke ? oe : ke;
        }
        if ((threadIdx.x & 63u) != 0) kb = ke = ~0ull;
    }
    if (kb != ~0ull && kb < __hip_atomic_load(&acc[s].bad, __ATOMIC_RELAXED, __HIP_MEMORY_SCOPE_AGENT)) atomicMin(&acc[s].bad, kb);
    if (ke != ~0ull && ke < __hip_atomic_load(&acc[s].end, __ATOMIC_RELAXED, __HIP_MEMORY_SCOPE_AGENT)) atomicMin(&acc[s].end, ke);
}

#define SRE_VERIFY_SPAN 1024u

__global__ __launch_bounds__(256) void
sre_k_verify_b(sre_scan_geom_t G, const sre_seg_summary_t *__restrict__ sum, VerifyAcc *__restrict__ acc)
{
    SRE_TAIL_PRIO();
    __shared__ unsigned long long sh_count, sh_ev, sh_sp;
    const uint64_t g0 = (uint64_t) blockIdx.x * SRE_VERIFY_SPAN;
    const uint64_t glast = (g0 + SRE_VERIFY_SPAN - 1 < G.nsegs) ? g0 + SRE_VERIFY_SPAN - 1 : G.nsegs - 1;
    const uint32_t s_first = stream_of(G, g0), s_last = stream_of(G, glast);
    const bool     uniform = (s_first == s_last);
    if (threadIdx.x == 0) {
        sh_count = 0;
        sh_ev = 0;
        sh_sp = 0;
    }
    __syncthreads();
    unsigned long long my_count = 0, my_ev = 0, my_sp = 0;
    for (uint32_t it = 0; it < SRE_VERIFY_SPAN / 256; it++) {
        const uint64_t g = g0 + it * 256u + threadIdx.x;
        if (g >= G.nsegs) break;
        const uint32_t s = uniform ? s_first : stream_of(G, g);
        const uint64_t k = g - geom_first(G, s);
        const uint64_t nseg = geom_first(G, s + 1) - geom_first(G, s);
        uint64_t       bad = acc[s].bad, end = acc[s].end;
        if (bad > nseg) bad = nseg;
        if (end > nseg) end = nseg;
        const uint64_t limit = end < bad ? end + 1 : bad;
        if (k < limit) {
            const sre_seg_summary_t &c = sum[g];
            if (uniform) {
                my_count += (unsigned long long) c.count;
                if (c.flags & SRE_SUM_LASTEV) my_ev = (unsigned long long) k + 1;
                if (c.cur_sp >= 0) my_sp = (unsigned long long) k + 1;
            } else {
                if (c.count) atomicAdd(&acc[s].count, (unsigned long long) c.count);
                if (c.flags & SRE_SUM_LASTEV) atomicMax(&acc[s].evseg, (unsigned long long) k + 1);
                if (c.cur_sp >= 0) atomicMax(&acc[s].spseg, (unsigned long long) k + 1);
            }
        }
    }
    if (uniform) {
        for (int d = 32; d >= 1; d >>= 1) {
            my_count += __shfl_down(my_count, d, 64);
            const unsigned long long e2 = __shfl_down(my_ev, d, 64), s2 = __shfl_down(my_sp, d, 64);
            my_ev = e2 > my_ev ? e2 : my_ev;
            my_sp = s2 > my_sp ? s2 : my_sp;
        }
        if ((threadIdx.x & 63u) == 0) {
            if (my_count) atomicAdd(&sh_count, my_count);
            if (my_ev) atomicMax(&sh_ev, my_ev);
            if (my_sp) atomicMax(&sh_sp, my_sp);
        }
    }
    __syncthreads();
    if (uniform && threadIdx.x == 0) {
        if (sh_count) atomicAdd(&acc[s_first].count, sh_count);
        if (sh_ev) atomicMax(&acc[s_first].evseg, sh_ev);
        if (sh_sp) atomicMax(&acc[s_first].spseg, sh_sp);
    }
}

__global__ __launch_bounds__(256) void
sre_k_verify_b2(sre_scan_geom_t G, const sre_seg_summary_t *__restrict__ sum, VerifyAcc *__restrict__ acc)
{
    SRE_TAIL_PRIO();
    __shared__ unsigned long long sh_max, sh_max_end;
    const uint64_t g0 = (uint64_t) blockIdx.x * SRE_VERIFY_SPAN;
    const uint64_t glast = (g0 + SRE_VERIFY_SPAN - 1 < G.nsegs) ? g0 + SRE_VERIFY_SPAN - 1 : G.nsegs - 1;
    const uint32_t s_first = stream_of(G, g0), s_last = stream_of(G, glast);
    const bool     uniform = (s_first == s_last);
    if (threadIdx.x == 0) sh_max = sh_max_end = 0;
    __syncthreads();
    unsigned long long mine = 0, mine_end = 0;
    for (uint32_t it = 0; it < SRE_VERIFY_SPAN / 256; it++) {
        const uint64_t g = g0 + it * 256u + threadIdx.x;
        if (g >= G.nsegs) break;
        const uint32_t s = uniform ? s_first : stream_of(G, g);
        const uint64_t k = g - geom_first(G, s);
        const uint64_t evseg = acc[s].evseg;
        const uint64_t nseg = geom_first(G, s + 1) - geom_first(G, s);
        if (!(sum[g].flags & SRE_SUM_STABLE)) {
            unsigned long long m1 = 0, m2 = 0;
            if (evseg != 0 && k + 1 < evseg) m1 = k + 1;
            if (k + 1 < nseg) m2 = k + 1;
            if (uniform) {
                mine = m1 > mine ? m1 : mine;
                mine_end = m2 > mine_end ? m2 : mine_end;
            } else {
                if (m1) atomicMax(&acc[s].unst, m1);
                if (m2) atomicMax(&acc[s].unst_end, m2);
            }
        }
    }
    if (uniform) {
        for (int d = 32; d >= 1; d >>= 1) {
            const unsigned long long o = __shfl_down(mine, d, 64), o2 = __shfl_down(mine_end, d, 64);
            mine = o > mine ? o : mine;
            mine_end = o2 > mine_end ? o2 : mine_end;
        }
        if ((threadIdx.x & 63u) == 0) {
            if (mine) atomicMax(&sh_max, mine);
            if (mine_end) atomicMax(&sh_max_end, mine_end);
        }
        __syncthreads();
        if (threadIdx.x == 0) {
            if (sh_max) atomicMax(&acc[s_first].unst, sh_max);
            if (sh_max_end) atomicMax(&acc[s_first].unst_end, sh_max_end);
        }
    }
}

#define SRE_EV_SP_SEARCH ((int64_t) -2)
__device__ inline sre_stream_status_t
assemble_status(const sre_scan_tables_t &T, const sre_seg_summary_t *__restrict__ sum, uint64_t nseg, const VerifyAcc &acc,
                bool defer_search = false)
{
    uint64_t       bad = acc.bad, end = acc.end;
    if (bad > nseg) bad = nseg;
    if (end > nseg) end = nseg;
    const bool     done = (end < bad) || (bad >= nseg);
    const uint64_t limit = end < bad ? end + 1 : bad;
    const uint64_t evseg = acc.evseg;

    sre_stream_status_t st;
    st.first_bad = (int64_t) bad;
    st.limit = (int64_t) limit;
    st.done = done ? 1 : 0;
    st.error = 0;
    st.need_maps = 0;
    st.pad = 0;
    st.count = (int64_t) acc.count;
    st.rc = RC_DECLINED;
    st.ev_pos = st.ev_sp = -1;
    st.ev_state = st.ev_sym = 0;
    st.ev_apos = -1;
    st.ev_astate = 0;
    st.valid_from = 0;
    st.ev_seg = -1;
    st.unst_seg = acc.unst ? (int64_t) acc.unst - 1 : -1;
    st.unst_end = acc.unst_end ? (int64_t) acc.unst_end - 1 : -1;
    if (done && evseg > 0) {
        const sre_seg_summary_t &c = sum[evseg - 1];
        st.ev_apos = c.lm_apos;
        st.ev_astate = c.lm_astate;
        st.ev_state = c.lm_state;
        st.ev_sym = c.lm_sym;
        st.ev_pos = c.lm_pos;
        st.ev_sp = c.lm_sp;
        st.ev_seg = (int64_t) evseg - 1;
        st.rc = T.trans[(size_t) c.lm_state * (T.ncls + 1) + c.lm_sym].regex;
        if (T.mode != SRE_HIP_PIKE_COUNT) st.count = 1;
        if (st.ev_sp < 0) {
            int64_t        sp = 0;
            const uint64_t spseg = acc.spseg;
            if (T.mode != SRE_HIP_PIKE_COUNT || spseg == 0) {
                sp = 0;
            } else if (spseg < evseg) {
                sp = sum[spseg - 1].cur_sp;
            } else if (defer_search) {
                sp = SRE_EV_SP_SEARCH;
            } else {
                for (int64_t q = (int64_t) evseg - 2; q >= 0; q--) {
                    if (sum[q].cur_sp >= 0) {
                        sp = sum[q].cur_sp;
                        break;
                    }
                }
            }
            st.ev_sp = sp;
        }
    }
    if (done && end < nseg && (sum[end].flags & SRE_SUM_ERROR)) st.error = 1;
    return st;
}

__global__ __launch_bounds__(64) void
sre_k_verify_c(sre_scan_tables_t T, sre_scan_geom_t G, const sre_seg_summary_t *__restrict__ sum,
               VerifyAcc *__restrict__ accs, sre_stream_status_t *__restrict__ status)
{
    SRE_TAIL_PRIO();
    const uint32_t s = blockIdx.x * blockDim.x + threadIdx.x;
    const bool     valid = s < G.nstreams;
    const uint32_t lane = threadIdx.x & 63u;
    sre_stream_status_t st;
    uint64_t            first = 0;
    st.ev_sp = -1;
    st.ev_seg = -1;
    if (valid) {
        const VerifyAcc acc = accs[s];
        accs[s].bad = accs[s].end = ~0ull;
        accs[s].count = accs[s].evseg = accs[s].spseg = accs[s].unst = accs[s].unst_end = 0;
        first = geom_first(G, s);
        const uint64_t nseg = geom_first(G, s + 1) - first;
        st = assemble_status(T, sum + first, nseg, acc, true);
    }
    uint64_t need = __builtin_amdgcn_ballot_w64(valid && st.ev_sp == SRE_EV_SP_SEARCH);
    while (need) {
        const int      l = __builtin_ctzll(need);
        need &= need - 1;
        const uint64_t f = __shfl(first, l, 64);
        const int64_t  top = __shfl(st.ev_seg, l, 64) - 1;
        int64_t        sp = 0;
        bool           found = false;
        for (int64_t hi = top; hi >= 0 && !found; hi -= 256) {
            int64_t v[4];
#pragma unroll
            for (int j = 0; j < 4; j++) {
                const int64_t q = hi - (int64_t) lane - 64 * j;
                v[j] = q >= 0 ? sum[f + (uint64_t) q].cur_sp : (int64_t) -1;
            }
#pragma unroll
            for (int j = 0; j < 4; j++) {
                const uint64_t b = __builtin_amdgcn_ballot_w64(v[j] >= 0);
                if (!found && b) {
                    sp = __shfl(v[j], __builtin_ctzll(b), 64);
                    found = true;
                }
            }
        }
        if ((int) lane == l) st.ev_sp = sp;
    }
    if (valid) status[s] = st;
}

#define SRE_VERIFY_ONE_MAX SRE_VERIFY_ONE_SEGS

template <int NT>
__device__ void
verify_one_stream(const sre_scan_tables_t &T, const sre_seg_summary_t *__restrict__ sum, uint64_t nseg,
                  sre_stream_status_t *__restrict__ status, VerifyAcc *sh_acc, sre_stream_status_t *out,
                  const sre_seg_digest_t *__restrict__ dig = nullptr)
{
    constexpr int  PER = SRE_VERIFY_ONE_MAX / NT;
    const uint32_t tid = threadIdx.x;
    if (tid == 0) {
        sh_acc->bad = sh_acc->end = ~0ull;
        sh_acc->count = sh_acc->evseg = sh_acc->spseg = sh_acc->unst = sh_acc->unst_end = 0;
    }
    uint32_t bits[PER], cnt[PER];
#pragma unroll
    for (int i = 0; i < PER; i++) {
        const uint64_t k = (uint64_t) i * NT + tid;
        bits[i] = 0;
        cnt[i] = 0;
        if (k < nseg && dig != nullptr) {
            const sre_seg_digest_t c = dig[k];
            const uint32_t         prev_out = k > 0 ? dig[k - 1].s_out : c.s_in;
            bits[i] = ((c.s_in == 0xffffffffu || c.s_in != prev_out) ? 1u : 0u) | c.bits;
            cnt[i] = c.count;
        } else if (k < nseg) {
            const sre_seg_summary_t &c = sum[k];
            const uint32_t s_in = c.s_in, fl = c.flags;
            const uint32_t prev_out = k > 0 ? sum[k - 1].s_out : s_in;
            bits[i] = ((s_in == 0xffffffffu || s_in != prev_out) ? 1u : 0u) | ((fl & SRE_SUM_TERM) ? 2u : 0u)
                      | ((fl & SRE_SUM_LASTEV) ? 4u : 0u) | (c.cur_sp >= 0 ? 8u : 0u) | ((fl & SRE_SUM_STABLE) ? 0u : 16u);
            cnt[i] = (uint32_t) c.count;
        }
    }
    __syncthreads();
    {
        unsigned long long bad = ~0ull, end = ~0ull;
#pragma unroll
        for (int i = PER - 1; i >= 0; i--) {
            const uint64_t k = (uint64_t) i * NT + tid;
            if (bits[i] & 1u) bad = k;
            if (bits[i] & 2u) end = k;
        }
        for (int d = 32; d >= 1; d >>= 1) {
            const unsigned long long b2 = __shfl_down(bad, d, 64), e2 = __shfl_down(end, d, 64);
            bad = b2 < bad ? b2 : bad;
            end = e2 < end ? e2 : end;
        }
        if ((tid & 63u) == 0) {
            if (bad != ~0ull) atomicMin(&sh_acc->bad, bad);
            if (end != ~0ull) atomicMin(&sh_acc->end, end);
        }
    }
    __syncthreads();
    {
        uint64_t bad = sh_acc->bad, end = sh_acc->end;
        if (bad > nseg) bad = nseg;
        if (end > nseg) end = nseg;
        const uint64_t     limit = end < bad ? end + 1 : bad;
        unsigned long long c = 0, ev = 0, sp = 0;
#pragma unroll
        for (int i = 0; i < PER; i++) {
            const uint64_t k = (uint64_t) i * NT + tid;
            if (k < limit) {
                c += cnt[i];
                if (bits[i] & 4u) ev = k + 1;
                if (bits[i] & 8u) sp = k + 1;
            }
        }
        for (int d = 32; d >= 1; d >>= 1) {
            c += __shfl_down(c, d, 64);
            const unsigned long long e2 = __shfl_down(ev, d, 64), s2 = __shfl_down(sp, d, 64);
            ev = e2 > ev ? e2 : ev;
            sp = s2 > sp ? s2 : sp;
        }
        if ((tid & 63u) == 0) {
            if (c) atomicAdd(&sh_acc->count, c);
            if (ev) atomicMax(&sh_acc->evseg, ev);
            if (sp) atomicMax(&sh_acc->spseg, sp);
        }
    }
    __syncthreads();
    {
        const uint64_t     evseg = sh_acc->evseg;
        unsigned long long mine = 0, mine_end = 0;
#pragma unroll
        for (int i = 0; i < PER; i++) {
            const uint64_t k = (uint64_t) i * NT + tid;
            if (k < nseg && (bits[i] & 16u)) {
                if (evseg != 0 && k + 1 < evseg) mine = k + 1;
                if (k + 1 < nseg) mine_end = k + 1;
            }
        }
        for (int d = 32; d >= 1; d >>= 1) {
            const unsigned long long o = __shfl_down(mine, d, 64), o2 = __shfl_down(mine_end, d, 64);
            mine = o > mine ? o : mine;
            mine_end = o2 > mine_end ? o2 : mine_end;
        }
        if ((tid & 63u) == 0) {
            if (mine) atomicMax(&sh_acc->unst, mine);
            if (mine_end) atomicMax(&sh_acc->unst_end, mine_end);
        }
    }
    __syncthreads();
    if (tid == 0) {
        *out = assemble_status(T, sum, nseg, *sh_acc);
        *status = *out;
    }
    __syncthreads();
}


__device__ inline int64_t
first_valid_segment(const sre_seg_summary_t *sum, int64_t sp, int64_t seg_bytes, int64_t ev_seg)
{
    for (int64_t k = sp / seg_bytes; k <= ev_seg; k++) {
        if (sum[k].cur_sp == sp) return k + 1;
    }
    return ev_seg + 1;
}

struct Tracer {
    const sre_scan_tables_t *T;
    const sre_seg_summary_t *sum;
    const uint8_t           *data;
    int64_t                  n, sp;
    uint32_t                 seg_bytes, init_state;
    int64_t                  apos;
    uint32_t                 astate;
    uint16_t                *ck;
    __attribute__((address_space(3))) uint16_t *trace;
    __attribute__((address_space(3))) uint8_t  *syms;
    int64_t                  seg_lo, seg_hi;
    int64_t                  blk_lo, blk_hi;
    int64_t                  valid_from;
    bool                     use_stable;
    uint32_t                 seg_entry;
    int64_t                  su_k = -1, su_lo = 0, su_hi = 0;
    uint32_t                 su_until = 0, su_s_in = 0;

#ifdef SRE_DEBUG_WALK
    unsigned long long dbg_seg_ticks = 0, dbg_blk_ticks = 0, dbg_entry_ticks = 0, dbg_top = 0, dbg_sb = 0, dbg_rest = 0;
    uint32_t           dbg_seg_calls = 0, dbg_blk_calls = 0, dbg_steps = 0;
#endif
    const __attribute__((address_space(3))) sre_dev_trans_t *ltrans;
    const __attribute__((address_space(3))) uint8_t         *lcls;
    uint32_t                                                  nsym;
    __device__ inline void bind()
    {
        ltrans = (const __attribute__((address_space(3))) sre_dev_trans_t *) (uintptr_t) T->trans;
        lcls = (const __attribute__((address_space(3))) uint8_t *) (uintptr_t) T->cls;
        nsym = T->ncls + 1;
    }

    __device__ __forceinline__ uint32_t step(uint32_t st, int64_t q) const
    {
        return ltrans[(size_t) st * nsym + lcls[data[q]]].next;
    }

    __device__ __forceinline__ uint32_t run_block(uint32_t cur, int64_t lo, uint32_t cnt, bool record)
    {
#ifdef SRE_DEBUG_WALK
        const unsigned long long dbg_t = wall_clock64();
        dbg_blk_calls++;
#endif
        const __attribute__((address_space(1))) uint8_t *g =
            (const __attribute__((address_space(1))) uint8_t *) (uintptr_t) (data + lo);
        if (cnt == 64 && (reinterpret_cast<uintptr_t>(data + lo) & 15) == 0) {
            typedef uint32_t u32x4 __attribute__((ext_vector_type(4)));
            const __attribute__((address_space(1))) u32x4 *gv = (const __attribute__((address_space(1))) u32x4 *) g;
            const u32x4 v0 = gv[0], v1 = gv[1], v2 = gv[2], v3 = gv[3];
            const uint32_t w[16] = {v0.x, v0.y, v0.z, v0.w, v1.x, v1.y, v1.z, v1.w,
                                    v2.x, v2.y, v2.z, v2.w, v3.x, v3.y, v3.z, v3.w};
#pragma unroll
            for (uint32_t x = 0; x < 64; x++) syms[x] = lcls[(w[x >> 2] >> ((x & 3) * 8)) & 0xffu];
        } else {
#pragma unroll 8
            for (uint32_t x = 0; x < cnt; x++) syms[x] = lcls[g[x]];
        }
        for (uint32_t x = 0; x < cnt; x++) {
            if (record) trace[x] = (uint16_t) cur;
            cur = ltrans[(size_t) cur * nsym + syms[x]].next;
        }
        if (record) trace[cnt] = (uint16_t) cur;
#ifdef SRE_DEBUG_WALK
        dbg_blk_ticks += wall_clock64() - dbg_t;
#endif
        return cur;
    }

    __device__ __forceinline__ uint32_t step16(uint32_t st, int64_t q) const
    {
        const uint32_t bits = T->class_bits, stride = T->stride;
        const uint4    v = *reinterpret_cast<const uint4 *>(data + q);
        const uint32_t words[4] = {v.x, v.y, v.z, v.w};
        uint32_t       so = st * SRE_FAST_ROW_BYTES, acc = 0;
        for (uint32_t j = 0; j < 16 / stride; j++) {
            uint32_t idx = 0;
            for (uint32_t u = 0; u < stride; u++) {
                const uint32_t b = j * stride + u;
                const uint32_t c = (words[b >> 2] >> ((b & 3) * 8)) & 0xffu;
                idx |= (bits == 8 ? c : (uint32_t) T->cls[c]) << (u * bits);
            }
            const uint32_t t = T->fast[(so >> 2) + idx];
            acc |= t;
            so = t & ~(SRE_FAST_ROW_BYTES - 1);
        }
        if (acc & SRE_FAST_SLOW) {
            for (int b = 0; b < 16; b++) st = step(st, q + b);
            return st;
        }
        return so / SRE_FAST_ROW_BYTES;
    }

    __device__ __forceinline__ uint32_t entry_state(int64_t kq) const
    {
        if (kq >= valid_from) return sum[kq].s_in & ~SRE_STATE_SKIP;
        uint32_t cur = init_state;
        for (int64_t q = sp; q < kq * (int64_t) seg_bytes; q++) cur = step(cur, q);
        return cur;
    }

    __device__ __forceinline__ void load_segment(int64_t kq, int64_t upto)
    {
#ifdef SRE_DEBUG_WALK
        const unsigned long long dbg_t = wall_clock64();
        dbg_seg_calls++;
#endif
        int64_t  lo = kq * (int64_t) seg_bytes, hi = lo + seg_bytes;
        uint32_t cur;
        if (hi > n) hi = n;
        if (((upto + 64) & ~(int64_t) 63) < hi) hi = (upto + 64) & ~(int64_t) 63;
        if (sp >= lo) {
            lo = sp;
            cur = init_state;
        } else {
#ifdef SRE_DEBUG_WALK
            const unsigned long long dbg_te = wall_clock64();
#endif
            cur = entry_state(kq);
#ifdef SRE_DEBUG_WALK
            dbg_entry_ticks += wall_clock64() - dbg_te;
#endif
            if (use_stable && kq >= valid_from) {
                int64_t skip = (int64_t) (sum[kq].stable_until & ~63u);
                if (skip > upto - lo) skip = (upto - lo) & ~(int64_t) 63;
                if (skip > 0 && lo + skip < hi) lo += skip;
            }
        }
        seg_lo = lo;
        seg_hi = hi;
        seg_entry = cur;
        const int64_t c0 = (lo + 63) & ~(int64_t) 63;
        int64_t       q = lo;
        const bool    aligned = (reinterpret_cast<uintptr_t>(data) & 15) == 0;
        if (q < c0 && q < hi) {
            const int64_t stop = c0 < hi ? c0 : hi;
            cur = run_block(cur, q, (uint32_t) (stop - q), false);
            q = stop;
        }
        uint32_t i = 0;
        while (q < hi) {
            ck[i++] = (uint16_t) cur;
            const int64_t stop = q + 64 < hi ? q + 64 : hi;
            if (aligned && stop - q == 64 && hi - q > 256) {
                for (int g4 = 0; g4 < 4; g4++) cur = step16(cur, q + 16 * g4);
            } else {
                cur = run_block(cur, q, (uint32_t) (stop - q), false);
            }
            q = stop;
        }
        ck[i] = (uint16_t) cur;
        blk_lo = 1;
        blk_hi = 0;
#ifdef SRE_DEBUG_WALK
        dbg_seg_ticks += wall_clock64() - dbg_t;
#endif
    }

    __device__ __forceinline__ uint32_t state_before(int64_t q)
    {
        if (q == sp) return init_state;
        if (use_stable && q > sp) {
            if (q - 1 < su_lo || q - 1 >= su_hi) {
                su_k = (q - 1) / seg_bytes;
                su_lo = su_k * (int64_t) seg_bytes;
                su_hi = su_lo + seg_bytes;
                su_until = sum[su_k].stable_until;
                su_s_in = sum[su_k].s_in;
            }
            const int64_t kq = su_k, sbase = su_lo;
            if (sbase >= sp && kq >= valid_from && q - sbase <= (int64_t) su_until) {
                return su_s_in & ~SRE_STATE_SKIP;
            }
        }
        if ((q < blk_lo || q > blk_hi) && apos >= 0 && q > apos && q <= apos + 64) {
            const int64_t hi = apos + 64 < n ? apos + 64 : n;
            run_block(astate, apos, (uint32_t) (hi - apos), true);
            blk_lo = apos;
            blk_hi = hi;
        }
        if (q < blk_lo || q > blk_hi) {
            if (q <= seg_lo || q > seg_hi) load_segment((q - 1) / seg_bytes, q);
            const int64_t c0 = (seg_lo + 63) & ~(int64_t) 63;
            int64_t       lo = (q - 1) & ~(int64_t) 63, hi;
            uint32_t      cur;
            if (lo < c0) {
                lo = seg_lo;
                cur = seg_entry;
                hi = c0 < seg_hi ? c0 : seg_hi;
            } else {
                cur = ck[(lo - c0) / 64];
                hi = lo + 64 < seg_hi ? lo + 64 : seg_hi;
            }
            run_block(cur, lo, (uint32_t) (hi - lo), true);
            blk_lo = lo;
            blk_hi = hi;
        }
        return trace[q - blk_lo];
    }

    __device__ __forceinline__ uint32_t sym_at(int64_t q) const
    {
        if (q >= blk_lo && q < blk_hi) return syms[q - blk_lo];
        return lcls[data[q]];
    }
};

__global__ __launch_bounds__(256) void
sre_k_lineage_maps(const sre_scan_tables_t *__restrict__ tabp, sre_scan_geom_t G,
                   const sre_seg_summary_t *__restrict__ sum,
                   const sre_stream_status_t *__restrict__ status,
                   sre_seg_lineage_t *__restrict__ maps)
{
    extern __shared__ __attribute__((aligned(16))) uint8_t lds[];
    const sre_scan_tables_t &T = *tabp;
    const uint32_t nsym = T.ncls + 1;
    uint8_t         *clsl = lds;
    sre_dev_trans_t *trl = reinterpret_cast<sre_dev_trans_t *>(lds + 256);
    const uint32_t   ntr = T.nstates * nsym;
    uint8_t         *parl = reinterpret_cast<uint8_t *>(trl + ntr);
    uint8_t         *flgl = parl + ((T.lin_total + 15u) & ~15u);
    for (uint32_t i = threadIdx.x; i < 256; i += blockDim.x) clsl[i] = T.cls[i];
    for (uint32_t i = threadIdx.x; i < ntr; i += blockDim.x) trl[i] = T.trans[i];
    for (uint32_t i = threadIdx.x; i < T.lin_total; i += blockDim.x) {
        parl[i] = T.lin_parent[i];
        flgl[i] = T.lin_flags[i];
    }
    __syncthreads();

    const uint64_t g = (uint64_t) blockIdx.x * blockDim.x + threadIdx.x;
    if (g >= G.nsegs) return;
    const uint32_t s = stream_of(G, g);
    const sre_stream_status_t &st = status[s];
    if (!st.need_maps) return;
    const uint64_t first = geom_first(G, s);
    const int64_t  k = (int64_t) (g - first);
    const int64_t  sp = st.ev_sp;
    if (k > st.ev_seg || (k + 1) * (int64_t) G.seg_bytes <= sp) return;

    const uint8_t *data = geom_ptr(G, s);
    const int64_t  n = (int64_t) geom_len(G, s);
    int64_t        lo = k * (int64_t) G.seg_bytes, hi = lo + G.seg_bytes;
    uint32_t       cur = sum[g].s_in & ~SRE_STATE_SKIP;
    if (hi > n) hi = n;
    if (k == st.ev_seg && st.ev_pos < hi) hi = st.ev_pos;
    if (sp >= lo) {
        lo = sp;
        cur = T.init[sp == 0 ? G.init_variant : restart_variant(T, data, sp)];
    } else if (k < (int64_t) st.valid_from) {
        cur = T.init[sp == 0 ? G.init_variant : restart_variant(T, data, sp)];
        for (int64_t x = sp; x < lo; x++) cur = trl[cur * nsym + clsl[data[x]]].next;
    }

    uint64_t anc = 0xfedcba9876543210ull;
    uint32_t saved = 0, stop = 0;
    uint32_t last_off = 0xffffffffu;
    auto step = [&](uint32_t c) {
        const sre_dev_trans_t &tr = trl[cur * nsym + clsl[c]];
        if (tr.pad && tr.lin_off == last_off) {
            cur = tr.next;
            return;
        }
        last_off = tr.lin_off;
        uint64_t nanc = 0;
        uint32_t nsaved = 0, nstop = 0;
        for (uint32_t j = 0; j < tr.lin_n; j++) {
            const uint32_t par = parl[tr.lin_off + j], f = flgl[tr.lin_off + j];
            if (par == 0xffu) {
                nstop |= 1u << j;
            } else {
                nanc |= ((anc >> (4 * par)) & 15ull) << (4 * j);
                nsaved |= (((saved >> par) & 1u) | (f & 1u)) << j;
                nstop |= (((stop >> par) & 1u) | ((f >> 1) & 1u)) << j;
            }
        }
        anc = nanc;
        saved = nsaved;
        stop = nstop;
        cur = tr.next;
    };
    int64_t q = lo;
    if ((reinterpret_cast<uintptr_t>(data) & 15) == 0) {
        for (; q < hi && (q & 63); q++) step(data[q]);
        uint4 nx[4];
        if (q + 64 <= hi) {
#pragma unroll
            for (int x = 0; x < 4; x++) nx[x] = *reinterpret_cast<const uint4 *>(data + q + 16 * x);
        }
        for (; q + 64 <= hi; q += 64) {
            uint4 v[4];
#pragma unroll
            for (int x = 0; x < 4; x++) v[x] = nx[x];
            if (q + 128 <= hi) {
#pragma unroll
                for (int x = 0; x < 4; x++) nx[x] = *reinterpret_cast<const uint4 *>(data + q + 64 + 16 * x);
            }
#pragma unroll
            for (int x = 0; x < 4; x++) {
                const uint32_t words[4] = {v[x].x, v[x].y, v[x].z, v[x].w};
#pragma unroll
                for (int b = 0; b < 16; b++) step((words[b >> 2] >> ((b & 3) * 8)) & 0xffu);
            }
        }
    }
    for (; q < hi; q++) step(data[q]);
    sre_seg_lineage_t out;
    out.anc = anc;
    out.saved = (uint16_t) saved;
    out.stop = (uint16_t) stop;
    out.pad = 0;
    maps[g] = out;
}

__global__ __launch_bounds__(256) void
sre_k_lineage_blocks(uint64_t nsegs, const sre_seg_lineage_t *__restrict__ maps,
                     sre_seg_lineage_t *__restrict__ blocks)
{
    const uint64_t t = (uint64_t) blockIdx.x * blockDim.x + threadIdx.x;
    const uint64_t b = t / 16;
    const uint32_t j = (uint32_t) (t % 16);
    const uint64_t g0 = b * SRE_LINEAGE_BLOCK;
    const bool     live = g0 + SRE_LINEAGE_BLOCK <= nsegs;
    uint32_t       cur = j;
    bool           bad = false;
    if (live) {
        for (int64_t g = (int64_t) (g0 + SRE_LINEAGE_BLOCK) - 1; g >= (int64_t) g0 && !bad; g--) {
            const sre_seg_lineage_t &m = maps[g];
            if (((m.saved | m.stop) >> cur) & 1u) bad = true;
            else cur = (uint32_t) ((m.anc >> (4 * cur)) & 15ull);
        }
    }
    uint64_t anc = (uint64_t) cur << (4 * j);
    uint32_t blocked = bad ? 1u << j : 0u;
    for (int d = 8; d >= 1; d >>= 1) {
        anc |= __shfl_down(anc, d, 16);
        blocked |= __shfl_down(blocked, d, 16);
    }
    if (live && j == 0) {
        sre_seg_lineage_t out;
        out.anc = anc;
        out.saved = (uint16_t) blocked;
        out.stop = 0;
        out.pad = 0;
        blocks[b] = out;
    }
}

struct LineageWalk {
    const sre_scan_tables_t *T;
    const sre_scan_tables_t *tabp;
    Tracer                  *tr;
    uint32_t                 variant;
    int64_t                  ev_seg, unst_seg;
    int64_t                  unst_end;
    uint64_t                 first;
    const sre_seg_lineage_t *maps, *blocks;
    bool                     use_maps;
    const int64_t           *carried;
    uint32_t                 carried_stride;
    int64_t                  base;
    int64_t                  walk_budget;

    __device__ __forceinline__ int run(int64_t p0, uint32_t j, uint32_t state_at_p0, uint64_t &unresolved, int64_t *vec)
    {
        const sre_scan_tables_t &T = *this->T;
        Tracer                  &tr = *this->tr;
        const uint32_t           nsym = T.ncls + 1;
        typedef const __attribute__((address_space(3))) uint32_t        *l_u32;
        typedef const __attribute__((address_space(3))) uint64_t        *l_u64;
        typedef const __attribute__((address_space(3))) uint8_t         *l_u8;
        typedef const __attribute__((address_space(3))) sre_dev_trans_t *l_tr;
        const l_u32    L_list_off = (l_u32) (uintptr_t) T.list_off, L_list_pcs = (l_u32) (uintptr_t) T.list_pcs;
        const l_u64    L_lin_saves = (l_u64) (uintptr_t) T.lin_saves;
        const l_u8     L_lin_parent = (l_u8) (uintptr_t) T.lin_parent;
        const l_tr     L_trans = (l_tr) (uintptr_t) T.trans;
        const uint32_t nslots = T.nslots, nstates = T.nstates;
        const uint64_t *const lin_early = tabp->lin_early;
        const int64_t  seg = (int64_t) tr.seg_bytes;
    const int64_t  k_sp = tr.sp / seg;
    const bool     can_jump = use_maps && T.max_threads <= 16;
    int64_t        budget = walk_budget;

    const uint16_t *const neutral = (T.mode == 1 && T.nshadow) ? tabp->neutral : nullptr;

    struct { uint32_t flags, s_in, s_out, stable_until, stable_from; } S = {0, 0, 0, 0, 0};
    int64_t S_k = -1, S_lo = -((int64_t) 1 << 40);

    for (int64_t p = p0; unresolved; p--) {
#ifdef SRE_DEBUG_WALK
        const unsigned long long dbg_a = wall_clock64();
#endif
        if (neutral != nullptr) {
            for (;;) {
                if (p <= tr.sp) break;
                if (p - 1 < S_lo || p - 1 >= S_lo + seg) {
                    S_k = (p - 1) / seg;
// ... 28 lines not shown
                    p = sbase + S.stable_from;
                    if (p < tr.sp) p = tr.sp;
                    continue;
                }
                break;
            }
        }
        if (can_jump && p > tr.sp && p % seg == 0 && p < p0) {
            int64_t k2 = p / seg - 1;
            while (k2 >= k_sp) {
                const uint64_t g2 = first + (uint64_t) k2;
                if (g2 % SRE_LINEAGE_BLOCK == SRE_LINEAGE_BLOCK - 1
                    && k2 - (int64_t) SRE_LINEAGE_BLOCK > k_sp)
                {
                    const sre_seg_lineage_t &bm = blocks[g2 / SRE_LINEAGE_BLOCK];
                    if (!((bm.saved >> j) & 1u)) {
                        j = (uint32_t) ((bm.anc >> (4 * j)) & 15ull);
                        k2 -= SRE_LINEAGE_BLOCK;
                        continue;
                    }
                }
                const sre_seg_lineage_t &m = maps[g2];
                if (((m.saved | m.stop) >> j) & 1u) break;
                j = (uint32_t) ((m.anc >> (4 * j)) & 15ull);
                k2--;
            }
            p = k2 < k_sp ? tr.sp : (k2 + 1) * seg;
        }
        if (!can_jump && --budget < 0 && T.max_threads <= 16) {
            return 1;
        }
#ifdef SRE_DEBUG_WALK
        const unsigned long long dbg_b = wall_clock64();
        tr.dbg_top += dbg_b - dbg_a;
#endif
        const uint32_t s_here = (p == p0) ? state_at_p0 : tr.state_before(p);
#ifdef SRE_DEBUG_WALK
        const unsigned long long dbg_c = wall_clock64();
        tr.dbg_sb += dbg_c - dbg_b;
#endif
#ifdef SRE_DEBUG_WALK
        tr.dbg_steps++;
#endif
#ifdef SRE_DEBUG_WALK_STEPS
        printf("walk p %lld s_here %u j %u pc %u unresolved %llx\n", (long long) p, s_here, j,
               T.list_pcs[T.list_off[s_here] + j], (unsigned long long) unresolved);
#endif
        if (L_list_pcs[L_list_off[s_here] + j] == 1) break;
        l_tr    t;
        int64_t val;
        if (p == tr.sp && carried != nullptr) {
            for (uint32_t q = 0; q < nslots; q++) {
                if ((unresolved >> q) & 1) vec[q] = carried[(size_t) j * carried_stride + q];
            }
            unresolved = 0;
            break;
        }
        if (p == tr.sp) {
            t = &L_trans[(size_t) nstates * nsym + variant];
            val = tr.sp;
        } else {
            const uint32_t s_prev = tr.state_before(p - 1);
            t = &L_trans[(size_t) s_prev * nsym + tr.sym_at(p - 1)];
            val = p;
        }
        const uint32_t lin = t->lin_off + j;
        const uint64_t m = L_lin_saves[lin] & unresolved;
        if (m) {
            for (uint32_t q = 0; q < nslots; q++) {
                if ((m >> q) & 1) vec[q] = val + base;
            }
            unresolved &= ~m;
        }
        if (lin_early != nullptr) {
            const uint64_t m2 = lin_early[lin] & unresolved;
            for (uint32_t q = 0; q < nslots; q++) {
                if ((m2 >> q) & 1) vec[q] = val - 1 + base;
            }
            unresolved &= ~m2;
        }
        if (p == tr.sp) break;
        j = L_lin_parent[lin];
        if (j == 0xffu) break;
#ifdef SRE_DEBUG_WALK
        tr.dbg_rest += wall_clock64() - dbg_c;
#endif
    }

        return 0;
    }
};

__device__ inline void
stage_walk_tables(const sre_scan_tables_t *__restrict__ tabp, uint8_t *lds, sre_scan_tables_t *Tsp)
{
    sre_scan_tables_t &Ts = *Tsp;
    {
        uint32_t *fast = reinterpret_cast<uint32_t *>(lds);
        uint8_t  *clsl = lds + tabp->fast_bytes;
        uint8_t  *trl = clsl + 256;
        const uint32_t tr_bytes = (tabp->nstates * (tabp->ncls + 1) + SRE_SCAN_NINIT) * (uint32_t) sizeof(sre_dev_trans_t);
        uint64_t *savl = reinterpret_cast<uint64_t *>(trl + tr_bytes);
        uint32_t *lofl = reinterpret_cast<uint32_t *>(savl + tabp->lin_total);
        uint32_t *lpcl = lofl + tabp->nstates + 1;
        uint8_t  *parl = reinterpret_cast<uint8_t *>(lpcl + tabp->list_total);
        if (threadIdx.x == 0) {
            Ts = *tabp;
            Ts.fast = fast;
            Ts.cls = clsl;
            Ts.trans = reinterpret_cast<const sre_dev_trans_t *>(trl);
            Ts.lin_saves = savl;
            Ts.lin_parent = parl;
            Ts.list_off = lofl;
            Ts.list_pcs = lpcl;
        }
        for (uint32_t i = threadIdx.x; i <= tabp->nstates; i += blockDim.x) lofl[i] = tabp->list_off[i];
        for (uint32_t i = threadIdx.x; i < tabp->list_total; i += blockDim.x) lpcl[i] = tabp->list_pcs[i];
        for (uint32_t i = threadIdx.x; i < tabp->lin_total; i += blockDim.x) {
            savl[i] = tabp->lin_saves[i];
            parl[i] = tabp->lin_parent[i];
        }
        for (uint32_t i = threadIdx.x; i < tabp->fast_bytes / 16; i += blockDim.x) {
            reinterpret_cast<uint4 *>(fast)[i] = reinterpret_cast<const uint4 *>(tabp->fast_plain)[i];
        }
        for (uint32_t i = threadIdx.x; i < tr_bytes / 8; i += blockDim.x) {
            reinterpret_cast<uint64_t *>(trl)[i] = reinterpret_cast<const uint64_t *>(tabp->trans)[i];
        }
        for (uint32_t i = threadIdx.x; i < 256; i += blockDim.x) clsl[i] = tabp->cls[i];
        __syncthreads();
    }
}

template <int NT>
__global__ __launch_bounds__(NT) void
sre_k_captures(const sre_scan_tables_t *__restrict__ tabp, sre_scan_geom_t G,
               const sre_seg_summary_t *__restrict__ sum,
               sre_stream_status_t *__restrict__ status, uint16_t *__restrict__ scratch,
               int64_t *__restrict__ records, uint32_t ovec_slots,
               const sre_seg_lineage_t *__restrict__ maps,
               const sre_seg_lineage_t *__restrict__ blocks, int use_maps)
{
    SRE_TAIL_PRIO();
    extern __shared__ __attribute__((aligned(16))) uint8_t lds[];
    __shared__ sre_scan_tables_t Ts;
    __shared__ uint16_t sh_trace[64][72];
    __shared__ uint8_t  sh_syms[64][72];
#ifdef SRE_DEBUG_WALK
    const unsigned long long dbg_t0 = wall_clock64();
#endif
    stage_walk_tables(tabp, lds, &Ts);
    if (NT != 64) {
        __shared__ VerifyAcc sh_acc;
        __shared__ sre_stream_status_t sh_st;
        verify_one_stream<NT>(Ts, sum, geom_first(G, 1), status, &sh_acc, &sh_st, G.digest);
    }
    const bool     lane_mode = NT == 64 && G.nstreams >= SRE_CAPTURE_LANE_STREAMS;
    if (!lane_mode && threadIdx.x != 0) return;
    const uint32_t wl = lane_mode ? threadIdx.x : 0u;
    auto one_stream = [&](const uint32_t s) {
    if (use_maps && !status[s].need_maps) return;
#ifdef SRE_DEBUG_WALK
    const unsigned long long dbg_ts = wall_clock64();
    unsigned long long       dbg_tw0 = 0, dbg_tw1 = 0;
#endif
    const sre_scan_tables_t   &T = Ts;
    const sre_stream_status_t  st = status[s];
    int64_t                   *rec = records + (size_t) s * (2 + ovec_slots);
    const uint32_t             nsym = T.ncls + 1;

    status[s].need_maps = 0;
    rec[0] = st.rc;
    rec[1] = st.count;
    for (uint32_t q = 0; q < ovec_slots; q++) rec[2 + q] = -1;
    if (!st.done) {
        rec[0] = RC_ERROR;
        return;
    }
    if (st.error && T.mode == SRE_HIP_PIKE_COUNT) rec[0] = RC_ERROR;
    if (st.ev_pos < 0) return;
    if (T.mode == 0) {
        rec[0] = 0;
        return;
    }

    Tracer tr;
    tr.T = &T;
    tr.sum = sum + geom_first(G, s);
    tr.data = geom_ptr(G, s);
    tr.n = (int64_t) geom_len(G, s);
    tr.sp = st.ev_sp;
    tr.seg_bytes = G.seg_bytes;
    const uint32_t variant = st.ev_sp == 0 ? G.init_variant : restart_variant(T, tr.data, st.ev_sp);
    tr.init_state = T.init[variant];
    tr.apos = (st.ev_apos >= st.ev_sp) ? st.ev_apos : -1;
    tr.astate = st.ev_astate;
    tr.ck = scratch + (size_t) s * (G.seg_bytes + 16);
    tr.trace = (__attribute__((address_space(3))) uint16_t *) sh_trace[wl];
    tr.syms = (__attribute__((address_space(3))) uint8_t *) sh_syms[wl];
    tr.bind();
    tr.seg_lo = tr.seg_hi = -1;
    tr.blk_lo = 1;
    tr.blk_hi = 0;
    tr.seg_entry = 0;
    tr.valid_from = first_valid_segment(tr.sum, tr.sp, (int64_t) G.seg_bytes, st.ev_seg);
    tr.use_stable = (T.mode == 1 && T.nshadow != 0);
    status[s].valid_from = (uint32_t) tr.valid_from;

    int64_t  vec[64];
    uint64_t unresolved = T.nslots >= 64 ? ~0ull : ((1ull << T.nslots) - 1);
    for (uint32_t q = 0; q < T.nslots; q++) vec[q] = -1;

    const sre_dev_trans_t &te = T.trans[(size_t) st.ev_state * nsym + st.ev_sym];
    uint32_t               j = te.src;
    if (te.kind == EV_DONE || te.kind == SRE_DEV_EV_DONE_EMPTY) {
        const uint64_t m = te.saves & unresolved;
        for (uint32_t q = 0; q < T.nslots; q++) {
            if ((m >> q) & 1) vec[q] = st.ev_pos + 1;
        }
        unresolved &= ~m;
    }
    if (te.early & unresolved) {
        const uint64_t m = te.early & unresolved;
        for (uint32_t q = 0; q < T.nslots; q++) {
            if ((m >> q) & 1) vec[q] = st.ev_pos;
        }
        unresolved &= ~m;
    }

    {
        LineageWalk lw;
        lw.T = &T;
        lw.tabp = tabp;
        lw.tr = &tr;
        lw.variant = variant;
        lw.ev_seg = st.ev_seg;
        lw.unst_seg = st.unst_seg;
        lw.unst_end = (int64_t) 1 << 62;
        lw.first = geom_first(G, s);
        lw.maps = maps;
        lw.blocks = blocks;
        lw.use_maps = use_maps != 0;
        lw.carried = nullptr;
        lw.carried_stride = 0;
        lw.base = 0;
        lw.walk_budget = SRE_WALK_BUDGET;
#ifdef SRE_DEBUG_WALK
        dbg_tw0 = wall_clock64();
#endif
        const int need = lw.run(st.ev_pos, j, st.ev_state, unresolved, vec);
#ifdef SRE_DEBUG_WALK
        dbg_tw1 = wall_clock64();
#endif
        if (need) {
            status[s].need_maps = 1;
            return;
        }
    }

    uint64_t ofs = 0;
    for (int64_t i = 0; i < st.rc; i++) ofs += T.multi_ncaps[i] + 1;
    ofs *= 2;
    const uint64_t ncopy = 2ull * (T.multi_ncaps[st.rc] + 1);
    for (uint64_t q = 0; q < ovec_slots; q++) rec[2 + q] = q < ncopy ? vec[ofs + q] : -1;
    rec[0] = (st.error && T.mode == SRE_HIP_PIKE_COUNT) ? RC_ERROR : st.rc;
#ifdef SRE_DEBUG_WALK
    printf("captures: stream %u (10 ns ticks) staging %llu, to the walk %llu, walk %llu, rest %llu; steps %u, load_segment %u calls %llu ticks "
           "(entry_state %llu), run_block %u calls %llu ticks; per step: top %llu, state_before(p) %llu, rest %llu\n", s,
           dbg_ts - dbg_t0, dbg_tw0 - dbg_ts, dbg_tw1 - dbg_tw0, wall_clock64() - dbg_tw1, tr.dbg_steps, tr.dbg_seg_calls,
           tr.dbg_seg_ticks, tr.dbg_entry_ticks, tr.dbg_blk_calls, tr.dbg_blk_ticks, tr.dbg_top, tr.dbg_sb, tr.dbg_rest);
#endif
    };
    if (lane_mode) {
        for (uint32_t s = blockIdx.x * 64u + wl; s < G.nstreams; s += gridDim.x * 64u) one_stream(s);
    } else {
        for (uint32_t s = blockIdx.x; s < G.nstreams; s += gridDim.x) one_stream(s);
    }
}


#define SRE_TAIL_THREADS 1024

struct TailCtxCompat {
    sre_stream_ctx_t *c;
    __device__ __forceinline__ uint32_t &state() const { return c->state; }
    __device__ __forceinline__ uint32_t &has_pending() const { return c->has_pending; }
    __device__ __forceinline__ int64_t  &pending_regex() const { return c->pending_regex; }
    __device__ __forceinline__ int64_t  *pending_vec() const { return c->pending_vec; }
    __device__ __forceinline__ int64_t  *caps() const { return &c->caps[0][0]; }
    __device__ __forceinline__ int64_t  *caps_next() const { return &c->caps_next[0][0]; }
    __device__ __forceinline__ uint32_t  stride() const { return SRE_STREAM_MAX_SLOTS; }
};
struct TailCtxRow {
    int64_t *row;
    uint32_t nslots, max_threads;
    __device__ __forceinline__ uint32_t &state() const { return reinterpret_cast<uint32_t *>(row + SRE_SROW_STATE)[0]; }
    __device__ __forceinline__ uint32_t &has_pending() const { return reinterpret_cast<uint32_t *>(row + SRE_SROW_STATE)[1]; }
    __device__ __forceinline__ int64_t  &pending_regex() const { return row[SRE_SROW_REGEX]; }
    __device__ __forceinline__ int64_t  *pending_vec() const { return row + SRE_SROW_HDR; }
    __device__ __forceinline__ int64_t  *caps() const { return row + SRE_SROW_HDR + nslots; }
    __device__ __forceinline__ int64_t  *caps_next() const { return row + SRE_SROW_HDR + nslots + (size_t) max_threads * nslots; }
    __device__ __forceinline__ uint32_t  stride() const { return nslots; }
};
struct TailChunk {
    const uint8_t           *data;
    int64_t                  n, base;
    const sre_seg_summary_t *sum;
    uint64_t                 nseg;
    uint32_t                 seg_bytes, variant, entry_state, ovec_slots;
    bool                     continues, eof;
    uint16_t                *scratch;
    __attribute__((address_space(3))) uint16_t *sh_trace;
    __attribute__((address_space(3))) uint8_t  *sh_syms;
};

template <class Ctx>
__device__ __forceinline__ int64_t
stream_tail_body(const sre_scan_tables_t &T, const sre_scan_tables_t *__restrict__ tabp, const sre_stream_status_t &st,
                 const TailChunk &K, const Ctx &ctx, sre_stream_result_t *__restrict__ res)
{
    int64_t                  rc_out = RC_ERROR;
    const sre_seg_summary_t *sum = K.sum;
    const uint64_t           nseg = K.nseg;
    const int64_t            base = K.base;
    const bool               eof = K.eof;
    const uint32_t           ovec_slots = K.ovec_slots;
    const uint32_t           nsym = T.ncls + 1;
    const bool               continues = K.continues;
    const int64_t            n = K.n;

    res->has_pending = 0;
    res->ev_in_chunk = 0;
    res->ev_slot1 = -1;
    res->poisoned = 0;
    res->next_state = 0;
    if (!continues) ctx.has_pending() = 0;
    if (!st.done) {
        rc_out = SRE_STREAM_UNSETTLED;
        return rc_out;
    }
    if (T.mode == 0) {
        const bool carried_match = continues && ctx.has_pending() != 0;
        bool       match_now = false, match_waits = false;
        if (carried_match) {
            match_now = n > 0 || eof;
            match_waits = !match_now;
        } else if (st.ev_pos >= 0) {
            const uint32_t kind = T.trans[(size_t) st.ev_state * (T.ncls + 1) + st.ev_sym].kind;
            const bool     listed_behind = (kind == EV_DONE || kind == SRE_DEV_EV_DONE_EMPTY);
            match_waits = listed_behind && st.ev_pos == n - 1 && !eof;
            match_now = !match_waits;
        }
        if (match_now) {
            rc_out = 0;
            ctx.state() = 0;
            ctx.has_pending() = 0;
        } else if (match_waits) {
            ctx.has_pending() = 1;
            ctx.state() = 1;
            res->next_state = 1;
            rc_out = -2;
        } else if (eof) {
            rc_out = RC_DECLINED;
            ctx.state() = 0;
            ctx.has_pending() = 0;
        } else {
            const uint32_t sF = sum[nseg - 1].s_out & ~SRE_STATE_SKIP;
            ctx.state() = tabp->unskip[sF];
            ctx.has_pending() = 0;
            res->next_state = ctx.state();
            rc_out = -2;
        }
        return rc_out;
    }

    Tracer tr;
    tr.T = &T;
    tr.sum = sum;
    tr.data = K.data;
    tr.n = n;
    tr.sp = 0;
    tr.seg_bytes = K.seg_bytes;
    const uint32_t variant = K.variant;
    tr.init_state = continues ? K.entry_state : T.init[variant];
    tr.apos = st.ev_apos >= 0 ? st.ev_apos : -1;
    tr.astate = st.ev_astate;
    tr.ck = K.scratch;
    tr.trace = K.sh_trace;
    tr.syms = K.sh_syms;
    tr.bind();
    tr.seg_lo = tr.seg_hi = -1;
    tr.blk_lo = 1;
    tr.blk_hi = 0;
    tr.seg_entry = 0;
    tr.valid_from = 1;
    tr.use_stable = (T.nshadow != 0);

    LineageWalk lw;
    lw.T = &T;
    lw.tabp = tabp;
    lw.tr = &tr;
    lw.variant = variant;
    lw.ev_seg = st.ev_seg >= 0 ? st.ev_seg : (int64_t) nseg;
    lw.unst_seg = st.ev_seg >= 0 ? st.unst_seg : (int64_t) nseg;
    lw.unst_end = T.nshadow ? st.unst_end : (int64_t) 1 << 62;
    lw.first = 0;
    lw.maps = lw.blocks = nullptr;
    lw.use_maps = false;
    lw.carried = continues ? ctx.caps() : nullptr;
    lw.carried_stride = ctx.stride();
    lw.base = base;
    lw.walk_budget = (int64_t) 1 << 62;

    const uint64_t all = T.nslots >= 64 ? ~0ull : ((1ull << T.nslots) - 1);
    int64_t        vec[SRE_STREAM_MAX_SLOTS];

    if (st.ev_pos >= 0) {
        uint64_t unresolved = all;
        for (uint32_t q = 0; q < T.nslots; q++) vec[q] = -1;
        const sre_dev_trans_t &te = T.trans[(size_t) st.ev_state * nsym + st.ev_sym];
        if (te.kind == EV_DONE || te.kind == SRE_DEV_EV_DONE_EMPTY) {
            const uint64_t m = te.saves & unresolved;
            for (uint32_t q = 0; q < T.nslots; q++) {
                if ((m >> q) & 1) vec[q] = st.ev_pos + 1 + base;
            }
            unresolved &= ~m;
        }
        if (te.early & unresolved) {
            const uint64_t m = te.early & unresolved;
            for (uint32_t q = 0; q < T.nslots; q++) {
                if ((m >> q) & 1) vec[q] = st.ev_pos + base;
            }
            unresolved &= ~m;
        }
            lw.run(st.ev_pos, te.src, st.ev_state, unresolved, vec);
        ctx.has_pending() = 1;
        ctx.pending_regex() = st.rc;
        for (uint32_t q = 0; q < T.nslots; q++) ctx.pending_vec()[q] = vec[q];
        res->ev_in_chunk = 1;
        res->ev_slot1 = vec[1];
    }

    const uint64_t last = (uint64_t) st.limit >= 1 ? (uint64_t) st.limit - 1 : 0;
    const bool     died = (sum[last].flags & SRE_SUM_TERM) != 0;
    if (died || eof) {
        if (ctx.has_pending()) {
            const int64_t id = ctx.pending_regex();
            uint64_t      ofs = 0;
            for (int64_t i = 0; i < id; i++) ofs += T.multi_ncaps[i] + 1;
            ofs *= 2;
            const uint64_t ncopy = 2ull * (T.multi_ncaps[id] + 1);
            for (uint64_t q = 0; q < ovec_slots && q < SRE_STREAM_MAX_SLOTS; q++) {
                res->ov[q] = q < ncopy ? ctx.pending_vec()[ofs + q] : -1;
            }
            rc_out = id;
            res->poisoned = st.error ? 1 : 0;
        } else {
            rc_out = RC_DECLINED;
        }
        ctx.state() = 0;
        ctx.has_pending() = 0;
        return rc_out;
    }

    const uint32_t sF = sum[nseg - 1].s_out & ~SRE_STATE_SKIP;
    const uint32_t nth = T.list_off[sF + 1] - T.list_off[sF];
    const uint32_t sNext = tabp->unskip[sF];
    int64_t        a0 = -1, a1 = -1;
    int64_t *fresh = ctx.caps_next();
    for (uint32_t j = 0; j < nth && j < SRE_STREAM_MAX_THREADS; j++) {
        uint64_t unresolved = all;
        for (uint32_t q = 0; q < T.nslots; q++) vec[q] = -1;
        lw.run(n, j, sF, unresolved, vec);
        for (uint32_t q = 0; q < T.nslots; q++) fresh[(size_t) j * ctx.stride() + q] = vec[q];
        uint64_t ofs = 0;
        for (uint32_t r = 0; r < T.nregexes; r++) {
            int64_t b = vec[ofs];
            if (b != -1 && (a0 == -1 || b < a0)) a0 = b;
            b = vec[1];
            if (b != -1 && (a1 == -1 || b > a1)) a1 = b;
            ofs += 2ull * (T.multi_ncaps[r] + 1);
        }
    }
    for (uint32_t j = 0; j < nth && j < SRE_STREAM_MAX_THREADS; j++) {
        for (uint32_t q = 0; q < T.nslots; q++) ctx.caps()[(size_t) j * ctx.stride() + q] = fresh[(size_t) j * ctx.stride() + q];
    }
    ctx.state() = sNext;
    res->next_state = sNext;
    res->ov[0] = a0;
    res->ov[1] = a1;
    rc_out = -2;
    if (ctx.has_pending()) {
        const int64_t id = ctx.pending_regex();
        uint64_t      ofs = 0;
        for (int64_t i = 0; i < id; i++) ofs += T.multi_ncaps[i] + 1;
        ofs *= 2;
        res->has_pending = 1;
        res->pending[0] = ctx.pending_vec()[ofs];
        res->pending[1] = ctx.pending_vec()[ofs + 1];
    }
    return rc_out;
}

__global__ __launch_bounds__(SRE_TAIL_THREADS) void
sre_k_stream_tail(const sre_scan_tables_t *__restrict__ tabp, sre_scan_geom_t G,
                  const sre_seg_summary_t *__restrict__ sum, sre_stream_status_t *__restrict__ status,
                  uint16_t *__restrict__ scratch, sre_stream_ctx_t *__restrict__ ctx,
                  sre_stream_result_t *__restrict__ res, int64_t base, int eof, uint32_t ovec_slots, int verify)
{
    SRE_TAIL_PRIO();
    extern __shared__ __attribute__((aligned(16))) uint8_t lds[];
    __shared__ sre_scan_tables_t Ts;
    __shared__ uint16_t sh_trace[72];
    __shared__ uint8_t  sh_syms[72];
    __shared__ VerifyAcc sh_acc;
    __shared__ sre_stream_status_t sh_st;
#ifdef SRE_DEBUG_TAIL
    const unsigned long long dbg_t0 = wall_clock64();
#endif
    stage_walk_tables(tabp, lds, &Ts);
#ifdef SRE_DEBUG_TAIL
    const unsigned long long dbg_t1 = wall_clock64();
#endif
    const uint64_t             nseg = geom_first(G, 1) - geom_first(G, 0);
    if (verify) verify_one_stream<SRE_TAIL_THREADS>(Ts, sum, nseg, status, &sh_acc, &sh_st, G.digest);
#ifdef SRE_DEBUG_TAIL
    const unsigned long long dbg_t2 = wall_clock64();
#endif
    if (threadIdx.x != 0) return;
    const sre_stream_status_t st = verify ? sh_st : status[0];
    TailChunk K;
    K.data = geom_ptr(G, 0);
    K.n = (int64_t) geom_len(G, 0);
    K.base = base;
    K.sum = sum;
    K.nseg = nseg;
    K.seg_bytes = G.seg_bytes;
    K.variant = G.init_variant;
    K.entry_state = G.entry_state;
    K.ovec_slots = ovec_slots;
    K.continues = (G.flags & SRE_GEOM_CONTINUES) != 0;
    K.eof = eof != 0;
    K.scratch = scratch;
    K.sh_trace = (__attribute__((address_space(3))) uint16_t *) sh_trace;
    K.sh_syms = (__attribute__((address_space(3))) uint8_t *) sh_syms;
    const TailCtxCompat C = {ctx};
    const int64_t rc_out = stream_tail_body(Ts, tabp, st, K, C, res);
#ifdef SRE_DEBUG_TAIL
    res->ov[SRE_STREAM_MAX_SLOTS - 3] = (int64_t) (dbg_t1 - dbg_t0);
    res->ov[SRE_STREAM_MAX_SLOTS - 2] = (int64_t) (dbg_t2 - dbg_t1);
    res->ov[SRE_STREAM_MAX_SLOTS - 1] = (int64_t) (wall_clock64() - dbg_t2);
#endif
    __threadfence_system();
    *reinterpret_cast<volatile int64_t *>(&res->rc) = rc_out;
}

__global__ __launch_bounds__(SRE_STREAMS_TAIL_THREADS) void
sre_k_streams_tail(const sre_scan_tables_t *__restrict__ tabp, sre_scan_geom_t G,
                   const sre_seg_summary_t *__restrict__ sum, const sre_stream_status_t *__restrict__ status,
                   uint16_t *__restrict__ scratch, int64_t *__restrict__ rows, sre_streams_layout_t L,
                   sre_stream_result_t *__restrict__ tailres, int64_t *__restrict__ recs,
                   sre_streams_info_t *__restrict__ info, int only_unsettled)
{
    SRE_TAIL_PRIO();
    extern __shared__ __attribute__((aligned(16))) uint8_t lds[];
    __shared__ sre_scan_tables_t Ts;
    __shared__ uint16_t sh_trace[72];
    __shared__ uint8_t  sh_syms[72];
    stage_walk_tables(tabp, lds, &Ts);
    if (threadIdx.x != 0) return;
    sre_stream_result_t *res = tailres + blockIdx.x;
    for (uint32_t s = blockIdx.x; s < G.nstreams; s += gridDim.x) {
        const uint64_t first = G.seg_first[s], nseg = G.seg_first[s + 1] - first;
        if (nseg == 0) continue;
        int64_t *rec = recs + (size_t) s * L.rec_slots;
        if (only_unsettled && rec[0] != SRE_STREAM_UNSETTLED) continue;
        int64_t       *row = rows + (size_t) s * L.row_words;
        const uint32_t e = G.sentry[s];
        uint64_t       fl = (uint64_t) row[SRE_SROW_FLAGS];
        const int64_t  processed = row[SRE_SROW_PROCESSED];
        TailChunk K;
        K.data = G.streams[s];
        K.n = (int64_t) G.lens[s];
        K.base = processed;
        K.sum = sum + first;
        K.nseg = nseg;
        K.seg_bytes = G.seg_bytes;
        K.variant = 0;
        K.entry_state = SRE_SENTRY_STATE(e);
        K.ovec_slots = L.ovec_slots;
        K.continues = (e & SRE_SENTRY_CONTINUES) != 0;
        K.eof = (e & SRE_SENTRY_NO_EOF) == 0;
        K.scratch = scratch + (size_t) blockIdx.x * (G.seg_bytes + 16);
        K.sh_trace = (__attribute__((address_space(3))) uint16_t *) sh_trace;
        K.sh_syms = (__attribute__((address_space(3))) uint8_t *) sh_syms;
        const TailCtxRow C = {row, L.nslots, L.max_threads};
        const int64_t rc = stream_tail_body(Ts, tabp, status[s], K, C, res);
        if (rc == SRE_STREAM_UNSETTLED) {
            rec[0] = rc;
            atomicAdd(reinterpret_cast<unsigned long long *>(&info->unsettled), 1ull);
            continue;
        }
        if (res->ev_in_chunk && res->ev_slot1 >= 0) {
            const int64_t p = res->ev_slot1 - processed;
            if (p > 0 && p <= K.n) {
                const uint8_t c = K.data[p - 1];
                const bool    word = (c >= '0' && c <= '9') || (c >= 'A' && c <= 'Z') || (c >= 'a' && c <= 'z') || c == '_';
                fl = (fl & ~(uint64_t) (SRE_SFL_NEWLINE | SRE_SFL_WORD)) | (c == '\n' ? SRE_SFL_NEWLINE : 0u)
                     | (word ? SRE_SFL_WORD : 0u);
            }
        }
        rec[0] = rc;
        rec[2] = 0;
        rec[3] = rec[4] = -1;
        for (uint32_t q = 0; q < L.ovec_slots; q++) rec[5 + q] = -1;
        if (rc == -2) {
            rec[1] = 0;
            if (L.ovec_slots >= 2 && Ts.mode != 0) {
                rec[5] = res->ov[0];
                rec[6] = res->ov[1];
            }
            if (res->has_pending) {
                rec[2] = 1;
                rec[3] = res->pending[0];
                rec[4] = res->pending[1];
            }
            row[SRE_SROW_PROCESSED] = processed + K.n;
            fl |= SRE_SFL_STARTED;
        } else {
            rec[1] = 1;
            if (rc >= 0 && Ts.mode != 0) {
                for (uint32_t q = 0; q < L.ovec_slots; q++) rec[5 + q] = res->ov[q];
            }
            fl = (fl & ~(uint64_t) SRE_SFL_STARTED) | SRE_SFL_CLOSED;
        }
        row[SRE_SROW_FLAGS] = (int64_t) fl;
    }
}

}

typedef void (*sre_scan_kernel_t)(const sre_scan_tables_t *, sre_scan_geom_t, sre_seg_summary_t *,
                                  const sre_stream_status_t *, const uint8_t *);

template <int MODE, bool GROW>
static sre_scan_kernel_t
scan_kernel_bits(uint32_t bits, bool wide4)
{
    switch (bits) {
    case 1: return sre_k_scan<MODE, 1, true, GROW>;
    case 2: return sre_k_scan<MODE, 2, true, GROW>;
    case 4: return (MODE == SRE_HIP_PIKE_COUNT && wide4) ? sre_k_scan<MODE, 4, (MODE == SRE_HIP_PIKE_COUNT), GROW>
                                                         : sre_k_scan<MODE, 4, false, GROW>;
    default: return sre_k_scan<MODE, 8, false, GROW>;
    }
}

static sre_scan_kernel_t
scan_kernel(const sre_scan_tables_t *h_tab)
{
    if (h_tab->mode != SRE_HIP_PIKE_COUNT) return scan_kernel_bits<1, false>(h_tab->class_bits, false);
    return h_tab->any_fresh ? scan_kernel_bits<SRE_HIP_PIKE_COUNT, true>(h_tab->class_bits, h_tab->wide != 0)
                            : scan_kernel_bits<SRE_HIP_PIKE_COUNT, false>(h_tab->class_bits, h_tab->wide != 0);
}

extern "C" size_t
sre_scan_lds_bytes(const sre_scan_tables_t *h_tab)
{
    const size_t tr = ((size_t) h_tab->nstates * (h_tab->ncls + 1) * 2 + 15) & ~(size_t) 15;
    const size_t half = (size_t) SRE_SCAN_ROUND * h_tab->class_bits / 8 * (h_tab->wide ? 2 : 1);
    static const char *pad_env = getenv("SRE_HIP_LDS_PAD");
    const size_t pad = pad_env ? (size_t) atoi(pad_env) : 0;
    size_t       need = pad + (size_t) h_tab->fast_rows * SRE_FAST_ROW_BYTES + 256 + tr + ((h_tab->nstates + 15u) & ~15u)
                        + 16 + (size_t) SRE_SCAN_BLOCK * (2 * half + 16);
    return need + (size_t) SRE_SCAN_BLOCK * 16;
}

extern "C" int
sre_scan_blocks_per_cu(const sre_scan_tables_t *h_tab)
{
    int          n = 0;
    const size_t shmem = sre_scan_lds_bytes(h_tab);
    hipError_t   e;
    e = hipOccupancyMaxActiveBlocksPerMultiprocessor(&n, scan_kernel(h_tab), SRE_SCAN_BLOCK, shmem);
    if (e != hipSuccess || n < 1) n = 1;
    if (n > 8) n = 8;
    return n;
}

extern "C" hipError_t
sre_launch_scan(const sre_scan_tables_t *d_tab, sre_scan_tables_t h_tab, sre_scan_geom_t geom,
                sre_seg_summary_t *d_sum, const sre_stream_status_t *d_lo, const uint8_t *d_entry,
                hipStream_t stream)
{
    if (geom.nsegs == 0) return hipSuccess;
    const uint32_t grid = (uint32_t) ((geom.nsegs + SRE_SCAN_BLOCK - 1) / SRE_SCAN_BLOCK);
    const size_t   shmem = sre_scan_lds_bytes(&h_tab);
    if (shmem > 48 * 1024) {
        static bool raised[2][9][2];
        bool       &done = raised[h_tab.mode == SRE_HIP_PIKE_COUNT][h_tab.class_bits & 8 ? 8 : h_tab.class_bits][h_tab.wide != 0];
        if (!done) {
            hipError_t e = hipFuncSetAttribute(reinterpret_cast<const void *>(scan_kernel(&h_tab)),
                                               hipFuncAttributeMaxDynamicSharedMemorySize,
                                               SRE_SCAN_LDS_LIMIT);
            if (e != hipSuccess) return e;
            done = true;
        }
    }
    hipLaunchKernelGGL(scan_kernel(&h_tab), dim3(grid), dim3(SRE_SCAN_BLOCK), shmem, stream,
                       d_tab, geom, d_sum, d_lo, d_entry);
    return hipGetLastError();
}

__global__ __launch_bounds__(256) void
sre_k_upload_words(const uint64_t *__restrict__ src, uint64_t *__restrict__ dst, uint32_t n)
{
    for (uint32_t i = blockIdx.x * 256u + threadIdx.x; i < n; i += gridDim.x * 256u) dst[i] = src[i];
}

extern "C" hipError_t
sre_launch_upload_words(const uint64_t *h_src_mapped, uint64_t *d_dst, uint32_t nwords, hipStream_t stream)
{
    if (nwords == 0) return hipSuccess;
    const uint32_t grid = (nwords + 255) / 256 < 64 ? (nwords + 255) / 256 : 64;
    hipLaunchKernelGGL(sre_k_upload_words, dim3(grid), dim3(256), 0, stream, h_src_mapped, d_dst, nwords);
    return hipGetLastError();
}

extern "C" size_t
sre_scan_verify_acc_bytes(uint32_t nstreams)
{
    return (size_t) nstreams * sizeof(VerifyAcc);
}

extern "C" hipError_t
sre_scan_verify_acc_init(void *d_acc, uint32_t nstreams, hipStream_t stream)
{
    hipError_t e = hipMemset2DAsync(d_acc, sizeof(VerifyAcc), 0xff, 2 * sizeof(unsigned long long),
// ... 168 lines not shown
```

Before: 6095 GB/s.

## Store compact per-segment digests and write full summaries only for non-plain segments

Segment summaries are now kept as a 16-byte digest for every segment. The full 136-byte summary is written only when a segment differs from the "plain" pass-through record, and readers rebuild plain records from the digest. The digest buffer is now allocated for any segment count, not just small ones, so verification and chaining kernels can read the compact digests everywhere. This is meant to cut summary write and read traffic for the roughly 254K segments of a 4 GiB stream. The cost is extra compare and pack work per segment and a branchier record-load path.

Measured after the change: 6261 GB/s, median of 6. 2.7% higher.

```diff
diff --git a/sregex_amd/csrc/sre_hip_batch.cpp b/sregex_amd/csrc/sre_hip_batch.cpp
--- a/sregex_amd/csrc/sre_hip_batch.cpp
+++ b/sregex_amd/csrc/sre_hip_batch.cpp
@@ -57,6 +57,7 @@
     uint64_t                 *d_seg_first, *h_seg_first;
     sre_seg_summary_t        *d_sum;
     sre_seg_digest_t         *d_digest;
+    uint64_t                  digest_cap;
     size_t                    sum_cap;
     sre_stream_status_t      *d_status, *h_status;
     void                     *d_acc;
@@ -932,11 +933,18 @@
         sc->sum_cap = nsegs;
     }
     sc->geom.digest = NULL;
-    if (nsegs <= SRE_VERIFY_ONE_SEGS && sc->mode != SRE_HIP_PIKE_COUNT) {
-        if (sc->d_digest == NULL
-            && hipMalloc(reinterpret_cast<void **>(&sc->d_digest), SRE_VERIFY_ONE_SEGS * sizeof(sre_seg_digest_t)) != hipSuccess)
-        {
+    if (sc->mode != SRE_HIP_PIKE_COUNT) {
+        if (nsegs > sc->digest_cap) {
+            const uint64_t want = nsegs > SRE_VERIFY_ONE_SEGS ? nsegs : SRE_VERIFY_ONE_SEGS;
+            if (sc->d_digest) (void) hipFree(sc->d_digest);
             sc->d_digest = NULL;
+            sc->digest_cap = 0;
+            if (hipMalloc(reinterpret_cast<void **>(&sc->d_digest), want * sizeof(sre_seg_digest_t)) == hipSuccess) {
+                sc->digest_cap = want;
+            } else {
+                sc->d_digest = NULL;
+                (void) hipGetLastError();
+            }
         }
         sc->geom.digest = sc->d_digest;
     }
@@ -1483,7 +1491,12 @@
         }
         const size_t ns = sc->geom.nsegs < 16 ? (size_t) sc->geom.nsegs : 16;
         std::vector<sre_seg_summary_t> hs(ns);
-        if (hipMemcpy(hs.data(), sc->d_sum, ns * sizeof(sre_seg_summary_t), hipMemcpyDeviceToHost) == hipSuccess) {
+        std::vector<sre_seg_digest_t>  hd(ns);
+        const bool                     dig = sc->geom.digest != NULL;
+        if (hipMemcpy(hs.data(), sc->d_sum, ns * sizeof(sre_seg_summary_t), hipMemcpyDeviceToHost) == hipSuccess
+            && (!dig || hipMemcpy(hd.data(), sc->geom.digest, ns * sizeof(sre_seg_digest_t), hipMemcpyDeviceToHost) == hipSuccess))
+        {
+            for (size_t k = 0; k < ns; k++) hs[k] = sre_scan_record_load(dig ? hd.data() : NULL, hs.data(), k, sc->geom.seg_bytes);
             for (size_t k = 0; k < ns; k++) {
                 fprintf(stderr, "[sregex-hip]   seg %zu: s_in %x s_out %x flags %x count %lld cur_sp %lld term %lld "
                                 "pe_pos %lld lm_pos %lld lm_sp %lld\n",
diff --git a/sregex_amd/csrc/sre_hip_scan.h b/sregex_amd/csrc/sre_hip_scan.h
--- a/sregex_amd/csrc/sre_hip_scan.h
+++ b/sregex_amd/csrc/sre_hip_scan.h
@@ -68,35 +68,7 @@
     const uint16_t        *neutral;
 } sre_scan_tables_t;
 
-typedef struct {
-    uint32_t s_in;
-    uint32_t s_out;
-    uint32_t flags;
-    uint32_t pad;
-    uint32_t pe_state, pe_sym;
-    int64_t  pe_pos, pe_sp;
-    uint32_t lm_state, lm_sym;
-    int64_t  lm_pos, lm_sp;
-    int64_t  lm_apos, pe_apos;
-    uint32_t lm_astate, pe_astate;
-    int64_t  term_pos;
-    int64_t  count;
-    int64_t  cur_sp;
-    int64_t  in_pe_pos;
-    uint32_t in_pe_state, in_pe_sym;
-    uint32_t stable_until, stable_from;
-} sre_seg_summary_t;
-
-typedef struct sre_seg_digest_s {
-    uint32_t s_in, s_out, bits, count;
-} sre_seg_digest_t;
-
-#define SRE_SUM_PENDING   1u
-#define SRE_SUM_TERM      2u
-#define SRE_SUM_LASTEV    4u
-#define SRE_SUM_ERROR     8u
-#define SRE_SUM_IN_PENDING 16u
-#define SRE_SUM_STABLE    32u
+#include "sre_scan_record.h"
 
 #define SRE_STATE_SKIP    0x40000000u
 
diff --git a/sregex_amd/csrc/sre_hip_scan.hip b/sregex_amd/csrc/sre_hip_scan.hip
--- a/sregex_amd/csrc/sre_hip_scan.hip
+++ b/sregex_amd/csrc/sre_hip_scan.hip
@@ -478,6 +478,22 @@
 #define SRE_COUNT_BLOCKS 3
 #endif
 
+#ifndef SRE_SCAN_COMPACT
+#define SRE_SCAN_COMPACT 1
+#endif
+
+template <int MODE>
+__device__ inline sre_seg_digest_t *
+scan_digest(const sre_scan_geom_t &G)
+{
+    return (SRE_SCAN_COMPACT && MODE != SRE_HIP_PIKE_COUNT) ? G.digest : nullptr;
+}
+__device__ inline sre_scan_records_t
+scan_records(const sre_scan_geom_t &G, const sre_seg_summary_t *sum)
+{
+    return sre_scan_records_t{sum, SRE_SCAN_COMPACT ? G.digest : nullptr, G.seg_bytes};
+}
+
 template <int MODE, int BITS, bool WIDE, bool GROW>
 __global__ __launch_bounds__(SRE_SCAN_BLOCK, MODE == SRE_HIP_PIKE_COUNT ? SRE_COUNT_BLOCKS : SRE_FIRST_BLOCKS) void
 sre_k_scan(const sre_scan_tables_t *__restrict__ tabp, sre_scan_geom_t G,
@@ -592,6 +608,7 @@
 
     int64_t  seg_a = 0, seg_b = 0;
     uint32_t s_in = 0, seed = 0;
+    const sre_scan_records_t rec{sum, scan_digest<MODE>(G), G.seg_bytes};
     int64_t  in_pe_pos = -1;
     uint32_t in_pe_state = 0, in_pe_sym = 0;
     bool     last_seg = false, warm = false;
@@ -614,7 +631,7 @@
                    : (G.flags & SRE_GEOM_CONTINUES) ? G.entry_state : T.init[G.init_variant];
             w.cur_sp = 0;
         } else if (lo_s >= 0 && (int64_t) k == lo_s) {
-            const sre_seg_summary_t &c = sum[g - 1];
+            const sre_seg_summary_t c = rec[g - 1];
             w.st = c.s_out & ~SRE_STATE_SKIP;
             w.set(F_SKIP_NEXT, MODE == SRE_HIP_PIKE_COUNT && (c.s_out & SRE_STATE_SKIP) != 0);
             w.cur_sp = c.cur_sp;
@@ -637,7 +654,7 @@
         } else if (entry != nullptr && entry[g] != 0xffu) {
             w.st = entry[g];
             if (MODE == SRE_HIP_PIKE_COUNT && lo_s > 0 && (T.state_flags[w.st] & 1)) {
-                const sre_seg_summary_t &c = sum[geom_first(G, sidx) + lo_s - 1];
+                const sre_seg_summary_t c = rec[geom_first(G, sidx) + lo_s - 1];
                 if (c.flags & SRE_SUM_PENDING) {
                     w.fl |= F_HAS_EV | F_IN_PENDING;
                     w.ev_state = c.pe_state;
@@ -656,7 +673,7 @@
             warm = true;
             seed = T.init[0];
             if (lo_s > 0) {
-                const sre_seg_summary_t &c = sum[geom_first(G, sidx) + lo_s - 1];
+                const sre_seg_summary_t c = rec[geom_first(G, sidx) + lo_s - 1];
                 const uint32_t           cs = c.s_out & ~SRE_STATE_SKIP;
                 if (cs != 0) {
                     if (!(MODE == SRE_HIP_PIKE_COUNT && (T.state_flags[cs] & 1))) {
@@ -1042,15 +1059,14 @@
     out.lm_astate = w.lm_astate;
     out.pe_apos = w.ev_apos;
     out.pe_astate = w.ev_astate;
-    sum[g] = out;
-    if (MODE != SRE_HIP_PIKE_COUNT && G.digest != nullptr) {
-        sre_seg_digest_t dg;
-        dg.s_in = out.s_in;
-        dg.s_out = out.s_out;
-        dg.bits = ((out.flags & SRE_SUM_TERM) ? 2u : 0u) | ((out.flags & SRE_SUM_LASTEV) ? 4u : 0u) | (out.cur_sp >= 0 ? 8u : 0u)
-                  | ((out.flags & SRE_SUM_STABLE) ? 0u : 16u);
-        dg.count = (uint32_t) out.count;
-        G.digest[g] = dg;
+    sre_seg_digest_t *const dig = scan_digest<MODE>(G);
+    if (dig != nullptr) {
+        bool                   plain;
+        const sre_seg_digest_t dg = sre_scan_record_pack(out, G.seg_bytes, &plain);
+        dig[g] = dg;
+        if (!plain) sum[g] = out;
+    } else {
+        sum[g] = out;
     }
 }
 
@@ -1178,7 +1194,7 @@
     if (s >= G.nstreams || status[s].done || status[s].first_bad < 1) return;
     const uint64_t first = geom_first(G, s), g_hi = geom_first(G, s + 1);
     uint64_t       g = first + (uint64_t) status[s].first_bad;
-    uint32_t       v = sum[g - 1].s_out & 63u;
+    uint32_t       v = scan_records(G, sum)[g - 1].s_out & 63u;
     while (g < g_hi) {
         if (g % SRE_FN_CHUNK == 0 && g + SRE_FN_CHUNK <= g_hi) {
             chunk_entry[g / SRE_FN_CHUNK] = (uint8_t) v;
@@ -1224,21 +1240,28 @@
     unsigned long long kb = ~0ull, ke = ~0ull;
     if (valid) {
         const uint64_t k = g - geom_first(G, s);
-        const uint32_t s_in = sum[g].s_in;
-        bool           bad = s_in == 0xffffffffu;
-        if (k > 0) {
-            const sre_seg_summary_t &p = sum[g - 1], &c = sum[g];
-            if (s_in != p.s_out) bad = true;
-            if (mode == SRE_HIP_PIKE_COUNT) {
-                const bool pp = (p.flags & SRE_SUM_PENDING) != 0, cp = (c.flags & SRE_SUM_IN_PENDING) != 0;
-                if (pp != cp) bad = true;
-                if (pp && cp && (p.pe_pos != c.in_pe_pos || p.pe_state != c.in_pe_state || p.pe_sym != c.in_pe_sym)) {
-                    bad = true;
+        const sre_seg_digest_t *const dig = mode == SRE_HIP_PIKE_COUNT ? nullptr : scan_records(G, sum).dig;
+        if (dig != nullptr) {
+            const sre_seg_digest_t c = dig[g];
+            if (c.s_in == 0xffffffffu || (k > 0 && c.s_in != dig[g - 1].s_out)) kb = k;
+            if (c.bits & SRE_DIGEST_TERM) ke = k;
+        } else {
+            const uint32_t s_in = sum[g].s_in;
+            bool           bad = s_in == 0xffffffffu;
+            if (k > 0) {
+                const sre_seg_summary_t &p = sum[g - 1], &c = sum[g];
+                if (s_in != p.s_out) bad = true;
+                if (mode == SRE_HIP_PIKE_COUNT) {
+                    const bool pp = (p.flags & SRE_SUM_PENDING) != 0, cp = (c.flags & SRE_SUM_IN_PENDING) != 0;
+                    if (pp != cp) bad = true;
+                    if (pp && cp && (p.pe_pos != c.in_pe_pos || p.pe_state != c.in_pe_state || p.pe_sym != c.in_pe_sym)) {
+                        bad = true;
+                    }
                 }
             }
-        }
-        if (bad) kb = k;
-        if (sum[g].flags & SRE_SUM_TERM) ke = k;
+            if (bad) kb = k;
+            if (sum[g].flags & SRE_SUM_TERM) ke = k;
+        }
     }
     const uint32_t s0 = (uint32_t) __builtin_amdgcn_readfirstlane((int) s);
     if (__builtin_amdgcn_ballot_w64(s != s0) == 0) {
@@ -1271,6 +1294,7 @@
     }
     __syncthreads();
     unsigned long long my_count = 0, my_ev = 0, my_sp = 0;
+    const sre_seg_digest_t *const dig = scan_records(G, sum).dig;
     for (uint32_t it = 0; it < SRE_VERIFY_SPAN / 256; it++) {
         const uint64_t g = g0 + it * 256u + threadIdx.x;
         if (g >= G.nsegs) break;
@@ -1282,15 +1306,27 @@
         if (end > nseg) end = nseg;
         const uint64_t limit = end < bad ? end + 1 : bad;
         if (k < limit) {
-            const sre_seg_summary_t &c = sum[g];
+            unsigned long long c_count;
+            bool               c_ev, c_sp;
+            if (dig != nullptr) {
+                const sre_seg_digest_t c = dig[g];
+                c_count = c.count;
+                c_ev = (c.bits & SRE_DIGEST_LASTEV) != 0;
+                c_sp = (c.bits & SRE_DIGEST_SP) != 0;
+            } else {
+                const sre_seg_summary_t &c = sum[g];
+                c_count = (unsigned long long) c.count;
+                c_ev = (c.flags & SRE_SUM_LASTEV) != 0;
+                c_sp = c.cur_sp >= 0;
+            }
             if (uniform) {
-                my_count += (unsigned long long) c.count;
-                if (c.flags & SRE_SUM_LASTEV) my_ev = (unsigned long long) k + 1;
-                if (c.cur_sp >= 0) my_sp = (unsigned long long) k + 1;
+                my_count += c_count;
+                if (c_ev) my_ev = (unsigned long long) k + 1;
+                if (c_sp) my_sp = (unsigned long long) k + 1;
             } else {
-                if (c.count) atomicAdd(&acc[s].count, (unsigned long long) c.count);
-                if (c.flags & SRE_SUM_LASTEV) atomicMax(&acc[s].evseg, (unsigned long long) k + 1);
-                if (c.cur_sp >= 0) atomicMax(&acc[s].spseg, (unsigned long long) k + 1);
+                if (c_count) atomicAdd(&acc[s].count, c_count);
+                if (c_ev) atomicMax(&acc[s].evseg, (unsigned long long) k + 1);
+                if (c_sp) atomicMax(&acc[s].spseg, (unsigned long long) k + 1);
             }
         }
     }
@@ -1327,6 +1363,7 @@
     if (threadIdx.x == 0) sh_max = sh_max_end = 0;
     __syncthreads();
     unsigned long long mine = 0, mine_end = 0;
+    const sre_seg_digest_t *const dig = scan_records(G, sum).dig;
     for (uint32_t it = 0; it < SRE_VERIFY_SPAN / 256; it++) {
         const uint64_t g = g0 + it * 256u + threadIdx.x;
         if (g >= G.nsegs) break;
@@ -1334,7 +1371,7 @@
         const uint64_t k = g - geom_first(G, s);
         const uint64_t evseg = acc[s].evseg;
         const uint64_t nseg = geom_first(G, s + 1) - geom_first(G, s);
-        if (!(sum[g].flags & SRE_SUM_STABLE)) {
+        if (dig != nullptr ? (dig[g].bits & SRE_DIGEST_UNSTABLE) != 0 : !(sum[g].flags & SRE_SUM_STABLE)) {
             unsigned long long m1 = 0, m2 = 0;
             if (evseg != 0 && k + 1 < evseg) m1 = k + 1;
             if (k + 1 < nseg) m2 = k + 1;
@@ -1367,7 +1404,7 @@
 
 #define SRE_EV_SP_SEARCH ((int64_t) -2)
 __device__ inline sre_stream_status_t
-assemble_status(const sre_scan_tables_t &T, const sre_seg_summary_t *__restrict__ sum, uint64_t nseg, const VerifyAcc &acc,
+assemble_status(const sre_scan_tables_t &T, const sre_scan_records_t sum, uint64_t nseg, const VerifyAcc &acc,
                 bool defer_search = false)
 {
     uint64_t       bad = acc.bad, end = acc.end;
@@ -1395,7 +1432,7 @@
     st.unst_seg = acc.unst ? (int64_t) acc.unst - 1 : -1;
     st.unst_end = acc.unst_end ? (int64_t) acc.unst_end - 1 : -1;
     if (done && evseg > 0) {
-        const sre_seg_summary_t &c = sum[evseg - 1];
+        const sre_seg_summary_t c = sum[evseg - 1];
         st.ev_apos = c.lm_apos;
         st.ev_astate = c.lm_astate;
         st.ev_state = c.lm_state;
@@ -1416,8 +1453,9 @@
                 sp = SRE_EV_SP_SEARCH;
             } else {
                 for (int64_t q = (int64_t) evseg - 2; q >= 0; q--) {
-                    if (sum[q].cur_sp >= 0) {
-                        sp = sum[q].cur_sp;
+                    const int64_t q_sp = sum[q].cur_sp;
+                    if (q_sp >= 0) {
+                        sp = q_sp;
                         break;
                     }
                 }
@@ -1447,7 +1485,7 @@
         accs[s].count = accs[s].evseg = accs[s].spseg = accs[s].unst = accs[s].unst_end = 0;
         first = geom_first(G, s);
         const uint64_t nseg = geom_first(G, s + 1) - first;
-        st = assemble_status(T, sum + first, nseg, acc, true);
+        st = assemble_status(T, scan_records(G, sum) + first, nseg, acc, true);
     }
     uint64_t need = __builtin_amdgcn_ballot_w64(valid && st.ev_sp == SRE_EV_SP_SEARCH);
     while (need) {
@@ -1462,7 +1500,7 @@
 #pragma unroll
             for (int j = 0; j < 4; j++) {
                 const int64_t q = hi - (int64_t) lane - 64 * j;
-                v[j] = q >= 0 ? sum[f + (uint64_t) q].cur_sp : (int64_t) -1;
+                v[j] = q >= 0 ? scan_records(G, sum)[f + (uint64_t) q].cur_sp : (int64_t) -1;
             }
 #pragma unroll
             for (int j = 0; j < 4; j++) {
@@ -1482,10 +1520,11 @@
 
 template <int NT>
 __device__ void
-verify_one_stream(const sre_scan_tables_t &T, const sre_seg_summary_t *__restrict__ sum, uint64_t nseg,
-                  sre_stream_status_t *__restrict__ status, VerifyAcc *sh_acc, sre_stream_status_t *out,
-                  const sre_seg_digest_t *__restrict__ dig = nullptr)
-{
+verify_one_stream(const sre_scan_tables_t &T, const sre_scan_records_t R, uint64_t nseg,
+                  sre_stream_status_t *__restrict__ status, VerifyAcc *sh_acc, sre_stream_status_t *out)
+{
+    const sre_seg_summary_t *const sum = R.sum;
+    const sre_seg_digest_t *const  dig = R.dig;
     constexpr int  PER = SRE_VERIFY_ONE_MAX / NT;
     const uint32_t tid = threadIdx.x;
     if (tid == 0) {
@@ -1583,7 +1622,7 @@
     }
     __syncthreads();
     if (tid == 0) {
-        *out = assemble_status(T, sum, nseg, *sh_acc);
+        *out = assemble_status(T, R, nseg, *sh_acc);
         *status = *out;
     }
     __syncthreads();
@@ -1591,7 +1630,7 @@
 
 
 __device__ inline int64_t
-first_valid_segment(const sre_seg_summary_t *sum, int64_t sp, int64_t seg_bytes, int64_t ev_seg)
+first_valid_segment(const sre_scan_records_t sum, int64_t sp, int64_t seg_bytes, int64_t ev_seg)
 {
     for (int64_t k = sp / seg_bytes; k <= ev_seg; k++) {
         if (sum[k].cur_sp == sp) return k + 1;
@@ -1601,7 +1640,7 @@
 
 struct Tracer {
     const sre_scan_tables_t *T;
-    const sre_seg_summary_t *sum;
+    sre_scan_records_t       sum;
     const uint8_t           *data;
     int64_t                  n, sp;
     uint32_t                 seg_bytes, init_state;
@@ -1841,7 +1880,7 @@
     const uint8_t *data = geom_ptr(G, s);
     const int64_t  n = (int64_t) geom_len(G, s);
     int64_t        lo = k * (int64_t) G.seg_bytes, hi = lo + G.seg_bytes;
-    uint32_t       cur = sum[g].s_in & ~SRE_STATE_SKIP;
+    uint32_t       cur = scan_records(G, sum)[g].s_in & ~SRE_STATE_SKIP;
     if (hi > n) hi = n;
     if (k == st.ev_seg && st.ev_pos < hi) hi = st.ev_pos;
     if (sp >= lo) {
@@ -2176,7 +2215,7 @@
     if (NT != 64) {
         __shared__ VerifyAcc sh_acc;
         __shared__ sre_stream_status_t sh_st;
-        verify_one_stream<NT>(Ts, sum, geom_first(G, 1), status, &sh_acc, &sh_st, G.digest);
+        verify_one_stream<NT>(Ts, scan_records(G, sum), geom_first(G, 1), status, &sh_acc, &sh_st);
     }
     const bool     lane_mode = NT == 64 && G.nstreams >= SRE_CAPTURE_LANE_STREAMS;
     if (!lane_mode && threadIdx.x != 0) return;
@@ -2209,7 +2248,7 @@
 
     Tracer tr;
     tr.T = &T;
-    tr.sum = sum + geom_first(G, s);
+    tr.sum = scan_records(G, sum) + geom_first(G, s);
     tr.data = geom_ptr(G, s);
     tr.n = (int64_t) geom_len(G, s);
     tr.sp = st.ev_sp;
@@ -2328,7 +2367,7 @@
 struct TailChunk {
     const uint8_t           *data;
     int64_t                  n, base;
-    const sre_seg_summary_t *sum;
+    sre_scan_records_t       sum;
     uint64_t                 nseg;
     uint32_t                 seg_bytes, variant, entry_state, ovec_slots;
     bool                     continues, eof;
@@ -2343,7 +2382,7 @@
                  const TailChunk &K, const Ctx &ctx, sre_stream_result_t *__restrict__ res)
 {
     int64_t                  rc_out = RC_ERROR;
-    const sre_seg_summary_t *sum = K.sum;
+    const sre_scan_records_t sum = K.sum;
     const uint64_t           nseg = K.nseg;
     const int64_t            base = K.base;
     const bool               eof = K.eof;
@@ -2546,7 +2585,7 @@
     const unsigned long long dbg_t1 = wall_clock64();
 #endif
     const uint64_t             nseg = geom_first(G, 1) - geom_first(G, 0);
-    if (verify) verify_one_stream<SRE_TAIL_THREADS>(Ts, sum, nseg, status, &sh_acc, &sh_st, G.digest);
+    if (verify) verify_one_stream<SRE_TAIL_THREADS>(Ts, scan_records(G, sum), nseg, status, &sh_acc, &sh_st);
 #ifdef SRE_DEBUG_TAIL
     const unsigned long long dbg_t2 = wall_clock64();
 #endif
@@ -2556,7 +2595,7 @@
     K.data = geom_ptr(G, 0);
     K.n = (int64_t) geom_len(G, 0);
     K.base = base;
-    K.sum = sum;
+    K.sum = scan_records(G, sum);
     K.nseg = nseg;
     K.seg_bytes = G.seg_bytes;
     K.variant = G.init_variant;
@@ -2606,7 +2645,7 @@
         K.data = G.streams[s];
         K.n = (int64_t) G.lens[s];
         K.base = processed;
-        K.sum = sum + first;
+        K.sum = scan_records(G, sum) + first;
         K.nseg = nseg;
         K.seg_bytes = G.seg_bytes;
         K.variant = 0;
diff --git a/sregex_amd/csrc/sre_scan_record.h b/sregex_amd/csrc/sre_scan_record.h
--- /dev/null
+++ b/sregex_amd/csrc/sre_scan_record.h
@@ -0,0 +1,127 @@
+#ifndef SRE_SCAN_RECORD_H
+#define SRE_SCAN_RECORD_H
+
+#include <stddef.h>
+#include <stdint.h>
+
+typedef struct {
+    uint32_t s_in;
+    uint32_t s_out;
+    uint32_t flags;
+    uint32_t pad;
+    uint32_t pe_state, pe_sym;
+    int64_t  pe_pos, pe_sp;
+    uint32_t lm_state, lm_sym;
+    int64_t  lm_pos, lm_sp;
+    int64_t  lm_apos, pe_apos;
+    uint32_t lm_astate, pe_astate;
+    int64_t  term_pos;
+    int64_t  count;
+    int64_t  cur_sp;
+    int64_t  in_pe_pos;
+    uint32_t in_pe_state, in_pe_sym;
+    uint32_t stable_until, stable_from;
+} sre_seg_summary_t;
+
+typedef struct sre_seg_digest_s {
+    uint32_t s_in, s_out, bits, count;
+} sre_seg_digest_t;
+
+#define SRE_SUM_PENDING   1u
+#define SRE_SUM_TERM      2u
+#define SRE_SUM_LASTEV    4u
+#define SRE_SUM_ERROR     8u
+#define SRE_SUM_IN_PENDING 16u
+#define SRE_SUM_STABLE    32u
+
+#ifdef __HIPCC__
+#define SRE_RECORD_FN static __host__ __device__ inline
+#else
+#define SRE_RECORD_FN static inline
+#endif
+
+#define SRE_DIGEST_TERM      2u
+#define SRE_DIGEST_LASTEV    4u
+#define SRE_DIGEST_SP        8u
+#define SRE_DIGEST_UNSTABLE  16u
+#define SRE_DIGEST_FULL      32u
+
+static_assert(sizeof(sre_seg_summary_t) == 136, "sre_seg_summary_t changed: update sre_scan_record_plain / _equal");
+
+SRE_RECORD_FN sre_seg_summary_t
+sre_scan_record_plain(uint32_t s_in, uint32_t seg_len)
+{
+    sre_seg_summary_t r;
+    r.s_in = s_in;
+    r.s_out = s_in;
+    r.flags = SRE_SUM_STABLE;
+    r.pad = 0;
+    r.pe_state = r.pe_sym = 0;
+    r.pe_pos = r.pe_sp = -1;
+    r.lm_state = r.lm_sym = 0;
+    r.lm_pos = r.lm_sp = -1;
+    r.lm_apos = r.pe_apos = -1;
+    r.lm_astate = r.pe_astate = 0;
+    r.term_pos = -1;
+    r.count = 0;
+    r.cur_sp = -1;
+    r.in_pe_pos = -1;
+    r.in_pe_state = r.in_pe_sym = 0;
+    r.stable_until = seg_len;
+    r.stable_from = 0;
+    return r;
+}
+
+SRE_RECORD_FN bool
+sre_scan_record_equal(const sre_seg_summary_t &a, const sre_seg_summary_t &b)
+{
+    return a.s_in == b.s_in && a.s_out == b.s_out && a.flags == b.flags && a.pad == b.pad
+           && a.pe_state == b.pe_state && a.pe_sym == b.pe_sym && a.pe_pos == b.pe_pos && a.pe_sp == b.pe_sp
+           && a.lm_state == b.lm_state && a.lm_sym == b.lm_sym && a.lm_pos == b.lm_pos && a.lm_sp == b.lm_sp
+           && a.lm_apos == b.lm_apos && a.pe_apos == b.pe_apos && a.lm_astate == b.lm_astate && a.pe_astate == b.pe_astate
+           && a.term_pos == b.term_pos && a.count == b.count && a.cur_sp == b.cur_sp
+           && a.in_pe_pos == b.in_pe_pos && a.in_pe_state == b.in_pe_state && a.in_pe_sym == b.in_pe_sym
+           && a.stable_until == b.stable_until && a.stable_from == b.stable_from;
+}
+
+SRE_RECORD_FN sre_seg_digest_t
+sre_scan_record_pack(const sre_seg_summary_t &x, uint32_t seg_len, bool *plain)
+{
+    sre_seg_digest_t d;
+    d.s_in = x.s_in;
+    d.s_out = x.s_out;
+    d.bits = ((x.flags & SRE_SUM_TERM) ? SRE_DIGEST_TERM : 0u) | ((x.flags & SRE_SUM_LASTEV) ? SRE_DIGEST_LASTEV : 0u)
+             | (x.cur_sp >= 0 ? SRE_DIGEST_SP : 0u) | ((x.flags & SRE_SUM_STABLE) ? 0u : SRE_DIGEST_UNSTABLE);
+    d.count = (uint32_t) x.count;
+    *plain = sre_scan_record_equal(x, sre_scan_record_plain(x.s_in, seg_len));
+    if (!*plain) d.bits |= SRE_DIGEST_FULL;
+    return d;
+}
+
+SRE_RECORD_FN sre_seg_summary_t
+sre_scan_record_load(const sre_seg_digest_t *dig, const sre_seg_summary_t *sum, uint64_t g, uint32_t seg_len)
+{
+    if (dig != NULL) {
+        const sre_seg_digest_t d = dig[g];
+        if (!(d.bits & SRE_DIGEST_FULL)) return sre_scan_record_plain(d.s_in, seg_len);
+    }
+    return sum[g];
+}
+
+#ifdef __HIPCC__
+struct sre_scan_records_t {
+    const sre_seg_summary_t *sum;
+    const sre_seg_digest_t  *dig;
+    uint32_t                 seg_len;
+    __host__ __device__ inline sre_seg_summary_t operator[](uint64_t k) const
+    {
+        return sre_scan_record_load(dig, sum, k, seg_len);
+    }
+    __host__ __device__ inline sre_scan_records_t operator+(uint64_t first) const
+    {
+        return sre_scan_records_t{sum + first, dig != NULL ? dig + first : NULL, seg_len};
+    }
+};
+#endif
+
+#endif
```
